# seqsense/pcgol

Hardware: AMD Instinct MI355X
Metric: Mpoints/sec ICP iter (corr+reduce) + kNN queries/sec, 1M-pt cloud (higher is better)
Workload: dtype f32

## Files before the change

pcgol_amd/csrc/icp.hip:

```cpp
#include <string.h>

#include <algorithm>
#include <array>
#include <chrono>
#include <condition_variable>
#include <mutex>
#include <string>
#include <thread>

#include <vector>

#include "knn_grid.h"
#include "knn_xwalk.h"
#include "icp_session_plan.h"
#include "icp_step_plan.h"
#include "strict_terms.h"
#include "gicp_terms.h"

namespace pcgx {

constexpr int kIcpBlock = kKnnBlock;

__device__ __forceinline__ double wave_sum_f64(double v) {
#pragma unroll
// ... 474 lines not shown
  if (kPlane) icp_plane_update_step(state, xchg, kp);
  else icp_update_step(state, xchg, kp);
}

__global__ __launch_bounds__(256) void pack_normals_kernel(const float *__restrict__ n3, int64_t n,
                                                           float4 *__restrict__ out) {
  const int64_t i = (int64_t)blockIdx.x * 256 + threadIdx.x;
  if (i < n) out[i] = make_float4(n3[3 * i], n3[3 * i + 1], n3[3 * i + 2], 0.0f);
}

__global__ __launch_bounds__(256) void pack_base_cov_kernel(const float *__restrict__ c6, int64_t n,
                                                            float4 *__restrict__ out) {
  const int64_t i = (int64_t)blockIdx.x * 256 + threadIdx.x;
  if (i >= n) return;
  out[2 * i] = make_float4(c6[6 * i], c6[6 * i + 1], c6[6 * i + 2], c6[6 * i + 3]);
  out[2 * i + 1] = make_float4(c6[6 * i + 4], c6[6 * i + 5], 0.0f, 0.0f);
}

__global__ __launch_bounds__(256) void gather_target_cov_kernel(const float *__restrict__ c6,
                                                                const int32_t *__restrict__ perm, int64_t n,
                                                                float2 *__restrict__ out) {
  const int64_t pos = (int64_t)blockIdx.x * 256 + threadIdx.x;
  if (pos >= n) return;
  const int64_t i = perm ? (int64_t)perm[pos] : pos;
  out[3 * pos] = make_float2(c6[6 * i], c6[6 * i + 1]);
  out[3 * pos + 1] = make_float2(c6[6 * i + 2], c6[6 * i + 3]);
  out[3 * pos + 2] = make_float2(c6[6 * i + 4], c6[6 * i + 5]);
}

__global__ __launch_bounds__(kGicpBlock) void icp_gicp_sums_kernel(
    const float *__restrict__ tx, const float *__restrict__ ty, const float *__restrict__ tz, int64_t nt,
    const IcpState *__restrict__ state, const float4 *__restrict__ match, const uint32_t *__restrict__ match_id,
    const float4 *__restrict__ base_cov, const float2 *__restrict__ target_cov, double *__restrict__ block_partials,
    uint32_t *__restrict__ dropped) {
  constexpr int NS = (int)P_COUNT;
  __shared__ double s_red[kGicpBlock / 64][NS];
  __shared__ uint32_t s_drop[kGicpBlock / 64];
  if (state->done) return;
  const bool project = state->iter > 0;
  float m[16];
#pragma unroll
  for (int i = 0; i < 16; i++) m[i] = project ? state->trans[i] : (i % 5 == 0 ? 1.0f : 0.0f);
  double acc[NS];
#pragma unroll
  for (int k = 0; k < NS; k++) acc[k] = 0.0;
  uint32_t n_drop = 0;
  const int64_t per = (nt + gridDim.x - 1) / gridDim.x;
  const int64_t r_begin = (int64_t)blockIdx.x * per;
  int64_t r_end = r_begin + per;
  if (r_end > nt) r_end = nt;
  for (int64_t i = r_begin + threadIdx.x; i < r_end; i += kGicpBlock) {
    const float4 bp = match[i];
    float x0 = tx[i], y0 = ty[i], z0 = tz[i];
    const float2 t0 = target_cov[3 * i], t1 = target_cov[3 * i + 1], t2 = target_cov[3 * i + 2];
    if (bp.w >= 0.0f) {
      const uint32_t id = match_id[i];
      const float4 c0 = base_cov[2 * (int64_t)id], c1 = base_cov[2 * (int64_t)id + 1];
      if (project) {
        float px, py, pz;
        mat4_transform(m, x0, y0, z0, px, py, pz);
        x0 = px; y0 = py; z0 = pz;
      }
      const float cb[6] = {c0.x, c0.y, c0.z, c0.w, c1.x, c1.y};
      const float ct[6] = {t0.x, t0.y, t1.x, t1.y, t2.x, t2.y};
      double e, g[6], H[21];
      if (gicp_terms(x0, y0, z0, bp.x, bp.y, bp.z, cb, ct, m, e, g, H)) {
        acc[P_VALUE] += e;
#pragma unroll
        for (int a = 0; a < 6; a++) acc[P_G0 + a] += g[a];
#pragma unroll
        for (int a = 0; a < 21; a++) acc[P_H0 + a] += H[a];
        acc[P_WEIGHT] += 1.0;
        acc[P_PAIRS] += 1.0;
      } else {
        n_drop++;
      }
    }
  }
  const int lane = threadIdx.x & 63, wave = threadIdx.x >> 6;
#pragma unroll
  for (int k = 0; k < NS; k++) {
    const double v = wave_sum_f64(acc[k]);
    if (lane == 0) s_red[wave][k] = v;
  }
#pragma unroll
  for (int o = 32; o > 0; o >>= 1) n_drop += __shfl_down(n_drop, o);
  if (lane == 0) s_drop[wave] = n_drop;
  __syncthreads();
  if (threadIdx.x < NS) {
    double v = 0.0;
    for (int w = 0; w < kGicpBlock / 64; w++) v += s_red[w][threadIdx.x];
    block_partials[(int64_t)blockIdx.x * NS + threadIdx.x] = v;
  }
  if (threadIdx.x == 0) {
    uint32_t d = 0;
    for (int w = 0; w < kGicpBlock / 64; w++) d += s_drop[w];
    dropped[blockIdx.x] = d;
  }
}

__global__ __launch_bounds__(256) void invert_positions_kernel(const uint32_t *__restrict__ pos_of, int64_t n,
                                                               uint32_t *__restrict__ orig_of) {
  const int64_t i = (int64_t)blockIdx.x * 256 + threadIdx.x;
  if (i < n) orig_of[pos_of[i]] = (uint32_t)i;
}

__global__ __launch_bounds__(256) void gather_soa_kernel(const float *__restrict__ q,
                                                         const int32_t *__restrict__ perm, int64_t n,
                                                         float *__restrict__ x, float *__restrict__ y,
                                                         float *__restrict__ z, uint32_t *__restrict__ pos_of) {
  const int64_t pos = (int64_t)blockIdx.x * 256 + threadIdx.x;
  if (pos >= n) return;
  const int64_t i = perm ? (int64_t)perm[pos] : pos;
  pos_of[i] = (uint32_t)pos;
  x[pos] = q[3 * i];
  y[pos] = q[3 * i + 1];
  z[pos] = q[3 * i + 2];
}

}

using namespace pcgx;

struct pcgx_icp_session {
  const pcgx_kdtree *base = nullptr;
  OwnedBlocks owned;
  bool patched = false;
  int64_t nt = 0;
  float *d_xyz = nullptr;
  IcpState *d_state = nullptr;
  double *d_partials = nullptr;
  uint32_t *d_pos_of = nullptr;
  uint32_t *d_orig_of = nullptr;
  float4 *d_match_caller = nullptr;
  bool caller_order_fresh = false;
  int strict = 0;
  bool strict_explicit = false;
  pcgx::StrictBuffers *strict_buf = nullptr;
  float *d_terms = nullptr;
  unsigned long long *d_valid = nullptr;
  int64_t nt_pad = 0;
  float4 *d_match = nullptr;
  float *d_match_cert = nullptr;
  uint32_t *d_first_leaf = nullptr;
  uint32_t *d_walk_list = nullptr;
  uint32_t *d_walk_count = nullptr;
  double *d_sums = nullptr;
  double *d_xchg = nullptr;
  int32_t steps_sharded = 0;
  int32_t host_iter = 0;
  bool spec_walk = true;
  bool spec_pending = false;
  hipStream_t spec_stream = nullptr;
  hipStream_t used[4] = {nullptr, nullptr, nullptr, nullptr};
  int n_used = 0;
  void touch(hipStream_t st) {
    for (int k = 0; k < n_used && k < 4; k++)
      if (used[k] == st) return;
    if (n_used > 0) (void)hipStreamSynchronize(used[0]);
    if (n_used < 4) used[n_used] = st;
    n_used++;
  }
  bool shard_failed = false;
  bool ring_fit_open = false;
  bool general_ready = true;
  bool small = false;
  int32_t *d_small_perm = nullptr;
  void *d_small_sync = nullptr;
  bool plane = false;
  uint32_t *d_match_id = nullptr;
  float4 *d_normals = nullptr;
  bool gicp = false;
  float4 *d_base_cov = nullptr;
  float2 *d_target_cov = nullptr;
  uint32_t *d_dropped = nullptr;
  int gicp_grid = 1;
  int n_sums() const { return plane ? (int)P_COUNT : (int)S_COUNT; }
  int grid = 1;
  IcpKernelParams kp;
  int32_t max_iteration = 20;
};

static pcgx_status settle(pcgx_icp_session *s, hipStream_t st);
static int icp_knob(const char *name, int def, int lo, int hi);

static pcgx_status enter(pcgx_icp_session *s, void *stream, hipStream_t *st) {
  *st = pick_stream(stream);
  s->touch(*st);
  return settle(s, *st);
}

template <class T>
static hipError_t session_alloc(pcgx_icp_session *s, T **p, size_t bytes) {
  const hipError_t e = dev_cache_alloc((void **)p, bytes);
  if (e == hipSuccess) s->owned.adopt(*p, dev_cache_free);
  return e;
}

static double now_us() { return std::chrono::duration<double, std::micro>(std::chrono::steady_clock::now().time_since_epoch()).count(); }

static IcpKernelParams make_kernel_params(const pcgx_icp_params *p) {
  IcpKernelParams kp;
  memset(&kp, 0, sizeof kp);
  kp.max_dist_sq = p->max_dist * p->max_dist;
  kp.min_dist_sq = p->min_dist_sq;
  kp.min_pairs = p->min_pairs == 0 ? 6 : p->min_pairs;
  kp.upd = resolve_updater(p->weight, p->threshold, p->max_iteration);
  kp.gn = resolve_gauss_newton(p->threshold, 0.0f, p->max_iteration);
  kp.weight_fn = p->weight_fn;
  kp.weight_a = p->weight_fn_param;
  return kp;
}

static int icp_grid(int64_t nt, const TreeView &tv) {
  int64_t blocks = (nt + kIcpBlock - 1) / kIcpBlock;
  int64_t cap = (int64_t)ctx().num_cu * walk_blocks_per_cu(tv) * walk_oversubscribe();
  if (blocks > cap) blocks = cap;
  if (blocks >= 8) blocks &= ~(int64_t)7;
  if (blocks < 1) blocks = 1;
  return (int)blocks;
}

struct IcpResetZero {
  uint32_t *p[3] = {nullptr, nullptr, nullptr};
  uint32_t words[3] = {0u, 0u, 0u};
};
__global__ void icp_reset_kernel(IcpState *__restrict__ state, IcpResetZero z) {
#pragma unroll
  for (int r = 0; r < 3; r++)
    for (uint32_t i = blockIdx.x * blockDim.x + threadIdx.x; i < z.words[r]; i += gridDim.x * blockDim.x) z.p[r][i] = 0u;
  if (threadIdx.x != 0 || blockIdx.x != 0) return;
  IcpState h;
  memset(&h, 0, sizeof h);
  const Mat4 id = mat4_translate(0.0f, 0.0f, 0.0f);
  for (int i = 0; i < 16; i++) h.trans[i] = id.m[i];
  *state = h;
}

static pcgx_status general_prepare(pcgx_icp_session *s, hipStream_t st) {
  if (s->general_ready) return PCGX_OK;
  const size_t n1 = (size_t)(s->nt ? s->nt : 1);
  PCGX_HIP_TRY(hipMemsetAsync(s->d_match, 0xFF, n1 * sizeof(float4), st));
  PCGX_HIP_TRY(hipMemsetAsync(s->d_match_cert, 0, n1 * sizeof(float), st));
  PCGX_HIP_TRY(hipMemsetAsync(s->d_first_leaf, 0, n1 * sizeof(uint32_t), st));
  PCGX_HIP_TRY(hipMemsetAsync(s->d_walk_count, 0, (size_t)s->grid * sizeof(uint32_t), st));
  s->general_ready = true;
  return PCGX_OK;
}

static pcgx_status reset_state(pcgx_icp_session *s, hipStream_t st) {
  IcpResetZero z;
  size_t zero_words = 0;
  if (s->spec_pending) {
    s->spec_pending = false;
    void *ptr[2];
    size_t bytes[2];
    strict_reset_ranges(s->strict_buf, ptr, bytes);
    if (s->d_walk_count) {
      z.p[0] = s->d_walk_count;
      z.words[0] = (uint32_t)s->grid;
    }
    for (int r = 0; r < 2; r++) {
      z.p[1 + r] = (uint32_t *)ptr[r];
      z.words[1 + r] = (uint32_t)(bytes[r] / sizeof(uint32_t));
    }
    for (int r = 0; r < 3; r++) zero_words += z.words[r];
  }
  const unsigned blocks = zero_words ? (unsigned)std::min<size_t>((zero_words + 1023) / 1024, 64) : 1u;
  hipLaunchKernelGGL(icp_reset_kernel, dim3(blocks), dim3(zero_words ? 256 : 64), 0, st, s->d_state, z);
  PCGX_HIP_TRY(hipGetLastError());
  s->host_iter = 0;
  if (s->shard_failed || s->steps_sharded > 0) {
    PCGX_TRY(strict_reset(s->strict_buf, st));
    s->shard_failed = false;
    s->steps_sharded = 0;
  }
  return PCGX_OK;
}

extern "C" pcgx_status pcgx_icp_session_reset(pcgx_icp_session *s, void *stream) {
  PCGX_API_LOCK();
  if (!s) return fail(PCGX_E_INVALID, "pcgx_icp_session_reset: NULL session");
  s->touch(pick_stream(stream));
  return reset_state(s, pick_stream(stream));
}

extern "C" pcgx_status pcgx_icp_session_set_pose(pcgx_icp_session *s, const float trans16[16],
                                                 int32_t iter, void *stream) {
  PCGX_API_LOCK();
  if (!s || !trans16 || iter < 0) return fail(PCGX_E_INVALID, "pcgx_icp_session_set_pose: bad argument");
  hipStream_t st;
  PCGX_TRY(enter(s, stream, &st));
  IcpState h;
  memset(&h, 0, sizeof h);
  memcpy(h.trans, trans16, sizeof h.trans);
  h.iter = iter;
  s->host_iter = 0;
  PCGX_HIP_TRY(hipMemcpyAsync(s->d_state, &h, sizeof h, hipMemcpyHostToDevice, st));
  PCGX_HIP_TRY(hipStreamSynchronize(st));
  return PCGX_OK;
}

extern "C" pcgx_status pcgx_icp_session_read_sums(pcgx_icp_session *s, double sums10[10], void *stream) {
  PCGX_API_LOCK();
  if (!s || !sums10) return fail(PCGX_E_INVALID, "pcgx_icp_session_read_sums: bad argument");
  if (s->plane) return fail(PCGX_E_INVALID, "pcgx_icp_session_read_sums: plane session (30 sums): use pcgx_icp_session_read_sums_n");
  hipStream_t st;
  PCGX_TRY(enter(s, stream, &st));
  PCGX_HIP_TRY(hipMemcpyAsync(sums10, s->d_sums, S_COUNT * sizeof(double), hipMemcpyDeviceToHost, st));
  PCGX_HIP_TRY(hipStreamSynchronize(st));
  return PCGX_OK;
}

extern "C" pcgx_status pcgx_icp_session_set_strict(pcgx_icp_session *s, int32_t on) {
  PCGX_API_LOCK();
  if (!s) return fail(PCGX_E_INVALID, "pcgx_icp_session_set_strict: NULL session");
  if (on && s->plane) return fail(PCGX_E_INVALID, "pcgx_icp_session_set_strict: point-to-plane sessions have no reference sums to reproduce");
  if (on < 0 || on > 2) return fail(PCGX_E_INVALID, "pcgx_icp_session_set_strict: mode must be 0, 1 or 2");
  if (s->spec_pending) PCGX_TRY(settle(s, s->spec_stream));
  s->strict = on;
  s->strict_explicit = on != 0;
  return PCGX_OK;
}

extern "C" pcgx_status pcgx_icp_session_sums_count(const pcgx_icp_session *s, int32_t *count) {
  PCGX_API_LOCK();
  if (!s || !count) return fail(PCGX_E_INVALID, "pcgx_icp_session_sums_count: bad argument");
  *count = s->n_sums();
  return PCGX_OK;
}

extern "C" pcgx_status pcgx_icp_session_read_sums_n(pcgx_icp_session *s, double *sums, int32_t cap, void *stream) {
  PCGX_API_LOCK();
  if (!s || !sums || cap < s->n_sums()) return fail(PCGX_E_INVALID, "pcgx_icp_session_read_sums_n: bad argument");
  hipStream_t st;
  PCGX_TRY(enter(s, stream, &st));
  PCGX_HIP_TRY(hipMemcpyAsync(sums, s->d_sums, (size_t)s->n_sums() * sizeof(double), hipMemcpyDeviceToHost, st));
  PCGX_HIP_TRY(hipStreamSynchronize(st));
  return PCGX_OK;
}

extern "C" pcgx_status pcgx_icp_session_free(pcgx_icp_session *s) {
  PCGX_API_LOCK();
  if (!s) return PCGX_OK;
  if (s->base) const_cast<pcgx_kdtree *>(s->base)->sessions.fetch_sub(1);
  if (s->n_used > 4) (void)hipDeviceSynchronize();
  else
    for (int k = 0; k < s->n_used; k++) (void)hipStreamSynchronize(s->used[k]);
  s->owned.release_all();
  delete s;
  return PCGX_OK;
}

static pcgx_status device_input(const float *src, size_t count, bool on_device, hipStream_t st, const float **d_out,
                                double *t_space = nullptr) {
  *d_out = src;
  if (on_device) return PCGX_OK;
  float *stage = nullptr;
  PCGX_TRY(ctx().arena.alloc_n(count, &stage));
  if (t_space) *t_space = now_us();
  PCGX_TRY(staged_upload(stage, src, count * sizeof(float), st));
  *d_out = stage;
  return PCGX_OK;
}

static pcgx_status setup_failed(hipError_t e) { return fail(PCGX_E_HIP, "icp session setup failed: %s", hipGetErrorString(e)); }

static pcgx_status session_allocate(pcgx_icp_session *s, const SessionPlan &p, double *d_sums) {
  void **const slot[kSessionBuffers] = {
      (void **)&s->d_xyz,        (void **)&s->d_state,      (void **)&s->d_partials,   (void **)&s->d_pos_of,
      (void **)&s->d_match,      (void **)&s->d_match_cert, (void **)&s->d_first_leaf, (void **)&s->d_walk_list,
      (void **)&s->d_walk_count, (void **)&s->d_sums,       (void **)&s->d_match_id,   (void **)&s->d_normals,
      (void **)&s->d_base_cov,   (void **)&s->d_target_cov, (void **)&s->d_dropped,    (void **)&s->d_valid,
      (void **)&s->d_small_perm};
  hipError_t e = hipSuccess;
  for (int b = 0; b < kSessionBuffers && e == hipSuccess; b++)
    if (p.bytes[b]) e = session_alloc(s, slot[b], p.bytes[b]);
  if (e == hipSuccess && p.small_buffers) e = session_alloc(s, &s->d_terms, small_fit_terms_bytes(s->nt));
  if (e == hipSuccess && p.small_buffers) e = session_alloc(s, &s->d_small_sync, small_fit_sync_bytes());
  if (e != hipSuccess) return fail(PCGX_E_OOM, "icp session allocation failed: %s", hipGetErrorString(e));
  if (d_sums) s->d_sums = d_sums;
  return PCGX_OK;
}

static pcgx_status stage_side_inputs(pcgx_icp_session *s, const float *normals, const float *base_cov6, bool on_device,
                                     hipStream_t st) {
  if (!s->plane) return PCGX_OK;
  const int64_t nb = s->base->n;
  hipError_t e;
  if (s->gicp && (e = hipMemsetAsync(s->d_dropped, 0, (size_t)s->gicp_grid * sizeof(uint32_t), st)) != hipSuccess)
    return setup_failed(e);
  PCGX_TRY(ctx().arena.begin(st));
  const float *d_in = nullptr;
  PCGX_TRY(device_input(s->gicp ? base_cov6 : normals, (size_t)nb * (s->gicp ? 6 : 3), on_device, st, &d_in));
  const dim3 blocks((unsigned)((nb + 255) / 256));
  if (s->gicp) hipLaunchKernelGGL(pack_base_cov_kernel, blocks, dim3(256), 0, st, d_in, nb, s->d_base_cov);
  else hipLaunchKernelGGL(pack_normals_kernel, blocks, dim3(256), 0, st, d_in, nb, s->d_normals);
  if ((e = hipStreamSynchronize(st)) != hipSuccess) return setup_failed(e);
  return PCGX_OK;
}

static pcgx_status order_target(pcgx_icp_session *s, const float *target, const float *target_cov6, bool on_device,
                                hipStream_t st, bool trace, double *t_phase) {
  const int64_t nt = s->nt;
  const pcgx_kdtree *base = s->base;
  Arena &ar = ctx().arena;
  PCGX_TRY(ar.begin(st));
  const float *d_q = nullptr;
  const void *up = nullptr;
  if (!on_device && s->small && (up = small_upload(target, (size_t)nt * 12)) != nullptr) {
    d_q = static_cast<const float *>(up);
    t_phase[2] = t_phase[3] = trace ? now_us() : 0.0;
  } else {
    PCGX_TRY(device_input(target, (size_t)nt * 3, on_device, st, &d_q, trace ? &t_phase[2] : nullptr));
    if (!on_device) t_phase[3] = trace ? now_us() : 0.0;
  }
  int32_t *perm = nullptr;
  if (s->small) {
    PCGX_TRY(small_fit_prepare(d_q, nt, base->bbox_lo, base->bbox_hi, s->d_small_perm, s->d_xyz, s->d_pos_of, s->d_state, s->d_terms,
                               s->d_small_sync, st));
    if (up) small_upload_read(st);
  } else {
    if (nt > 1) {
      PCGX_TRY(ar.alloc_n((size_t)nt, &perm));
      PCGX_TRY(morton_order(d_q, nt, base->bbox_lo, base->bbox_hi, perm, st));
    }
    hipLaunchKernelGGL(gather_soa_kernel, dim3((unsigned)((nt + 255) / 256)), dim3(256), 0, st, d_q, perm, nt,
                       s->d_xyz, s->d_xyz + nt, s->d_xyz + 2 * nt, s->d_pos_of);
  }
  if (s->gicp) {
    const float *d_c6 = nullptr;
    PCGX_TRY(device_input(target_cov6, (size_t)nt * 6, on_device, st, &d_c6));
    hipLaunchKernelGGL(gather_target_cov_kernel, dim3((unsigned)((nt + 255) / 256)), dim3(256), 0, st, d_c6,
                       (const int32_t *)perm, nt, s->d_target_cov);
  }
  t_phase[4] = trace ? now_us() : 0.0;
  const hipError_t e = hipGetLastError();
  return e == hipSuccess ? PCGX_OK : setup_failed(e);
}

static SessionFacts session_facts(const pcgx_kdtree *base, bool normals, bool covariances, const pcgx_icp_params *params,
                                  int64_t nt, bool caller_sums) {
  static_assert(PCGX_SUMS_REFERENCE == 0 && PCGX_SUMS_F64_TREE == 1 && S_COUNT == 10 && P_COUNT == 30,
                "SessionFacts::sums_mode, SessionPlan::n_sums");
  static const bool small_on = icp_knob("PCGX_ICP_SMALL", 1, 0, 1) != 0;
  SessionFacts f;
  f.normals = normals;
  f.covariances = covariances;
  f.sums_mode = params->sums_mode;
  if (const char *e = getenv("PCGX_ICP_STRICT")) f.strict_override = e[0] == '1' ? 1 : (e[0] == '2' ? 2 : 0);
  f.nt = nt;
  f.n_base = base->n;
  f.patched = base->n_deleted > 0;
  f.has_nan = base->has_nan;
  f.small_on = small_on;
  f.small_eligible = small_fit_eligible(base->view(), nt, base->many_ties);
  f.small_wants_order = small_fit_wants_order(nt);
  f.grid = icp_grid(nt, base->view());
  f.num_cu = ctx().num_cu;
  f.caller_sums = caller_sums;
  f.state_bytes = sizeof(IcpState);
  return f;
}

static pcgx_status session_create(const pcgx_kdtree *base, const float *normals, float damping,
                                  const float *target, int64_t nt, int32_t target_on_device,
                                  const pcgx_icp_params *params, double *d_sums,
                                  pcgx_icp_session **out, const float *base_cov6 = nullptr,
                                  const float *target_cov6 = nullptr) {
  if (!out) return fail(PCGX_E_INVALID, "pcgx_icp_session_create: out is NULL");
  *out = nullptr;
  if (!base || !params || nt < 0 || (nt > 0 && !target))
    return fail(PCGX_E_INVALID, "pcgx_icp_session_create: bad argument");
  if (params->weight_fn < 0 || params->weight_fn >= PCGX_WEIGHT_KINDS)
    return fail(PCGX_E_INVALID, "pcgx_icp_session_create: weight_fn %d is none of the built-in forms (a custom Go closure "
                                "cannot run on the device)", params->weight_fn);
  if (normals && params->weight_fn != PCGX_WEIGHT_ONE)
    return fail(PCGX_E_INVALID, "the point-to-plane extension takes the default weight only");
  if (base_cov6 && params->weight_fn != PCGX_WEIGHT_ONE)
    return fail(PCGX_E_INVALID, "the GICP extension takes the default weight only");
  if (params->sums_mode < 0 || params->sums_mode >= PCGX_SUMS_KINDS)
    return fail(PCGX_E_INVALID, "pcgx_icp_session_create: sums_mode %d is none of PCGX_SUMS_*", params->sums_mode);
  PCGX_TRY(ensure_init());
  hipStream_t st = ctx().stream;
  const bool patched = base->n_deleted > 0;
  if (patched && base->n_deleted >= base->n)
    return fail(PCGX_E_NOT_ENOUGH_PAIRS, "not enough correspondence pairs (every base point was deleted)");
  static const bool trace = getenv("PCGX_FIT_TRACE") != nullptr;
  double t_phase[6] = {0, 0, 0, 0, 0, 0};
  t_phase[0] = trace ? now_us() : 0.0;

  const SessionFacts f = session_facts(base, normals != nullptr, base_cov6 != nullptr, params, nt, d_sums != nullptr);
  const SessionPlan p = plan_session(f);

  pcgx_icp_session *s = new pcgx_icp_session();
  s->base = base;
  s->touch(st);
  s->patched = f.patched;
  const_cast<pcgx_kdtree *>(base)->sessions.fetch_add(1);
  s->nt = nt;
  s->nt_pad = p.nt_pad;
  s->gicp = p.gicp;
  s->plane = p.plane;
  s->strict = p.strict;
  s->strict_explicit = p.strict_explicit;
  s->small = p.small;
  s->grid = f.grid;
  s->gicp_grid = p.gicp_grid;
  s->kp = make_kernel_params(params);
  s->kp.gn.damping = damping;
  s->max_iteration = s->kp.upd.max_iteration;
  s->general_ready = false;

  pcgx_status rc = session_allocate(s, p, d_sums);
  if (rc == PCGX_OK) rc = stage_side_inputs(s, normals, base_cov6, target_on_device != 0, st);
  t_phase[1] = trace ? now_us() : 0.0;
  if (rc == PCGX_OK && p.start_values) rc = reset_state(s, st);
  if (rc == PCGX_OK && p.start_values) rc = general_prepare(s, st);
  if (rc == PCGX_OK && nt > 0) rc = order_target(s, target, target_cov6, target_on_device != 0, st, trace, t_phase);
  if (rc != PCGX_OK) {
    pcgx_icp_session_free(s);
    return rc;
  }
  if (trace)
    fprintf(stderr, "pcgx session trace: buffers %.0f us, memsets + arena %.0f, upload %.0f, order + gather enqueued %.0f\n",
            t_phase[1] - t_phase[0], t_phase[2] - t_phase[1], t_phase[3] - t_phase[2], t_phase[4] - t_phase[3]);
  *out = s;
  return PCGX_OK;
}

extern "C" pcgx_status pcgx_icp_session_create(const pcgx_kdtree *base, const float *target,
                                               int64_t nt, int32_t target_on_device,
                                               const pcgx_icp_params *params, double *d_sums10,
                                               pcgx_icp_session **out) {
  PCGX_API_LOCK();
  return session_create(base, nullptr, 0.0f, target, nt, target_on_device, params, d_sums10, out);
}

extern "C" pcgx_status pcgx_icp_plane_session_create(const pcgx_kdtree *base, const float *base_normals,
                                                     const float *target, int64_t nt, int32_t on_device,
                                                     const pcgx_icp_params *params, float damping,
                                                     double *d_sums30, pcgx_icp_session **out) {
  PCGX_API_LOCK();
  if (!base_normals) return fail(PCGX_E_INVALID, "pcgx_icp_plane_session_create: base_normals is NULL");
  if (params && params->min_dist_sq > 0.0f)
    return fail(PCGX_E_INVALID, "pcgx_icp_plane_session_create: MinDistSq > 0 (approximate search) is not offered here");
  if (!(damping >= 0.0f)) return fail(PCGX_E_INVALID, "pcgx_icp_plane_session_create: damping must be >= 0");
  return session_create(base, base_normals, damping, target, nt, on_device, params, d_sums30, out);
}

extern "C" pcgx_status pcgx_icp_gicp_session_create(const pcgx_kdtree *base, const float *base_cov6, const float *target,
                                                    const float *target_cov6, int64_t nt, int32_t on_device,
                                                    const pcgx_icp_params *params, float damping, double *d_sums30,
                                                    pcgx_icp_session **out) {
  PCGX_API_LOCK();
  if (!base_cov6 || (nt > 0 && !target_cov6))
    return fail(PCGX_E_INVALID, "pcgx_icp_gicp_session_create: a covariance array is NULL");
  if (params && params->min_dist_sq > 0.0f)
    return fail(PCGX_E_INVALID, "pcgx_icp_gicp_session_create: MinDistSq > 0 (approximate search) is not offered here");
  if (!(damping >= 0.0f)) return fail(PCGX_E_INVALID, "pcgx_icp_gicp_session_create: damping must be >= 0");
  return session_create(base, nullptr, damping, target, nt, on_device, params, d_sums30, out, base_cov6, target_cov6);
}

extern "C" pcgx_status pcgx_icp_gicp_session_dropped(pcgx_icp_session *s, void *stream, int64_t *n) {
  PCGX_API_LOCK();
  if (!s || !n) return fail(PCGX_E_INVALID, "pcgx_icp_gicp_session_dropped: bad argument");
  if (!s->gicp) return fail(PCGX_E_INVALID, "pcgx_icp_gicp_session_dropped: not a GICP session");
  hipStream_t st;
  PCGX_TRY(enter(s, stream, &st));
  std::vector<uint32_t> h((size_t)s->gicp_grid);
  PCGX_HIP_TRY(hipMemcpyAsync(h.data(), s->d_dropped, h.size() * sizeof(uint32_t), hipMemcpyDeviceToHost, st));
  PCGX_HIP_TRY(hipStreamSynchronize(st));
  int64_t sum = 0;
  for (uint32_t v : h) sum += (int64_t)v;
  *n = sum;
  return PCGX_OK;
}

static int icp_knob(const char *name, int def, int lo, int hi) {
  if (const char *e = getenv(name)) {
    const int v = atoi(e);
    if (v >= lo && v <= hi) return v;
  }
  return def;
}

static const StepKnobs &step_knobs() {
  static const StepKnobs knobs = [] {
    StepKnobs k;
    k.tight = icp_knob("PCGX_ICP_TIGHT", 32, 0, 32);
    k.chunks = icp_knob("PCGX_ICP_CHUNKS", 2, 1, 64);
    k.left_blocks = icp_knob("PCGX_ICP_LEFTOVER_BLOCKS", 128, 8, 4096) & ~7;
    k.cert_on = icp_knob("PCGX_ICP_CERT", 1, 0, 1) != 0;
    k.spec_on = icp_knob("PCGX_ICP_SPEC_WALK", 1, 0, 1) != 0;
    k.fused_from = icp_knob("PCGX_ICP_FUSED_FROM", 2, 0, 1 << 30);
    k.test_force_walk = icp_knob("PCGX_TEST_ICP_FORCE_WALK", 0, 0, 1 << 30);
    k.test_fused_search = icp_knob("PCGX_TEST_ICP_FUSED_SEARCH", 0, 0, 1 << 30);
    k.test_fused_grid_walk = icp_knob("PCGX_TEST_ICP_FUSED_GRID_WALK", 0, 0, 1 << 30);
    return k;
  }();
  return knobs;
}

static pcgx_status ensure_strict_buf(pcgx_icp_session *s, hipStream_t st) {
  if (s->strict_buf) return PCGX_OK;
  PCGX_TRY(strict_create(s->nt, s->d_xyz, s->d_xyz + s->nt, s->d_xyz + 2 * s->nt, (const uint32_t *)s->d_pos_of, &s->strict_buf, st));
  s->owned.adopt(s->strict_buf, [](void *p) { strict_destroy(static_cast<StrictBuffers *>(p)); });
  return PCGX_OK;
}

static pcgx_status decide_step(pcgx_icp_session *s, hipStream_t st, bool may_speculate, StepPlan *plan) {
  if (!s->patched && s->base->n_deleted > 0) s->patched = true;
  PCGX_TRY(general_prepare(s, st));
  StepFacts f;
  f.caller_had_pairs = s->caller_order_fresh;
  s->caller_order_fresh = false;
  if (!s->patched && s->strict == 1 && !s->plane && s->nt > 0) {
    if (!s->d_match_caller) {
      hipError_t e = session_alloc(s, &s->d_orig_of, (size_t)s->nt * sizeof(uint32_t));
      if (e == hipSuccess) e = session_alloc(s, &s->d_match_caller, (size_t)s->nt * sizeof(float4));
      if (e != hipSuccess) {
        (void)hipGetLastError();
        s->owned.give_up(s->d_orig_of);
        s->owned.give_up(s->d_match_caller);
        s->d_orig_of = nullptr;
        s->d_match_caller = nullptr;
      } else {
        hipLaunchKernelGGL(invert_positions_kernel, dim3((unsigned)((s->nt + 255) / 256)), dim3(256), 0, st,
                           (const uint32_t *)s->d_pos_of, s->nt, s->d_orig_of);
      }
    }
    PCGX_TRY(ensure_strict_buf(s, st));
    f.exchange = strict_work(s->strict_buf, s->kp)->exchange;
  }
  f.patched = s->patched;
  f.plane = s->plane;
  f.strict = s->strict;
  f.min_dist = s->kp.min_dist_sq > 0.0f;
  f.has_targets = s->nt > 0;
  f.grid_enabled = grid_enabled(s->base);
  f.has_cert = s->base->grid.cert != nullptr;
  f.have_match_caller = s->d_match_caller != nullptr;
  f.spec_walk = s->spec_walk;
  f.host_iter = s->host_iter;
  f.may_speculate = may_speculate;
  f.grid = s->grid;
  *plan = plan_step(f, step_knobs());
  s->caller_order_fresh = plan->next_caller_had_pairs;
  if (plan->no_walk) {
    s->spec_pending = true;
    s->spec_stream = st;
  }
  return PCGX_OK;
}

static pcgx_status enqueue_corr_patched(pcgx_icp_session *s, hipStream_t st) {
  XTreeView xv;
  PCGX_TRY(xtree_view(s->base, &xv, st));
  const size_t lds = (size_t)(xv.depth > 1 ? xv.depth : 2) * kIcpBlock * sizeof(uint32_t);
  const int64_t guard = xwalk_guard(s->base->n);
  const float *x = s->d_xyz, *y = s->d_xyz + s->nt, *z = s->d_xyz + 2 * s->nt;
  ProfScope prof(PCGX_PROF_ICP_WALK, st);
  const auto launch = [&](auto kernel) {
    hipLaunchKernelGGL(kernel, dim3(s->grid), dim3(kIcpBlock), lds, st, xv, x, y, z, s->nt, s->d_state, s->kp, s->d_match,
                       s->d_partials, s->d_match_id, (const float4 *)s->d_normals, guard);
  };
  const bool min_dist = s->kp.min_dist_sq > 0.0f;
  if (s->gicp) launch(icp_corr_xkernel<false, true, false>);
  else if (s->plane) launch(icp_corr_xkernel<false, true>);
  else if (min_dist && s->strict) launch(icp_corr_xkernel<true, false, false>);
  else if (min_dist) launch(icp_corr_xkernel<true, false>);
  else if (s->strict) launch(icp_corr_xkernel<false, false, false>);
  else launch(icp_corr_xkernel<false, false>);
  PCGX_HIP_TRY(hipGetLastError());
  return PCGX_OK;
}

static pcgx_status enqueue_corr(pcgx_icp_session *s, hipStream_t st, const StepPlan &p) {
  if (p.corr == kCorrPatched) return enqueue_corr_patched(s, st);
  if (p.corr == kCorrNone) return PCGX_OK;
  const StepKnobs &k = step_knobs();
  const float *x = s->d_xyz, *y = s->d_xyz + s->nt, *z = s->d_xyz + 2 * s->nt;
  const uint32_t *orig_of = p.write_caller ? s->d_orig_of : nullptr;
  float4 *match_caller = p.write_caller ? s->d_match_caller : nullptr;
  float *cert = p.cert ? s->d_match_cert : nullptr;
  const bool grid = p.corr != kCorrWalk;
  if (grid) {
    ProfScope prof_grid(PCGX_PROF_ICP_GRID, st);
    const bool strict_grid = s->strict && !s->plane;
    const auto launch = [&](auto kernel, int block) {
      hipLaunchKernelGGL(kernel, dim3(xcd_grid((unsigned)((s->nt + block - 1) / block))), dim3(block), 0, st, s->base->grid, x,
                         y, z, s->nt, s->d_state, s->kp, s->d_match, s->d_match_id, (const float4 *)s->d_normals,
                         s->d_first_leaf, s->d_walk_list, s->d_walk_count, (uint32_t)p.n_corr, s->d_partials,
                         (unsigned long long *)nullptr, orig_of, match_caller, cert, p.grid_has_caller_pairs ? 1 : 0,
                         p.no_walk ? 0 : 1, strict_grid ? k.test_force_walk : 0);
    };
    if (s->gicp) launch(icp_grid_kernel<true, false, false>, kIcpGridBlock);
    else if (s->plane) launch(icp_grid_kernel<true>, kIcpGridBlock);
    else if (s->strict) launch(icp_grid_kernel<false, false, false>, kIcpStrictGridBlock);
    else launch(icp_grid_kernel<false>, kIcpGridBlock);
  }
  if (p.corr == kCorrGrid) return PCGX_OK;
  ProfScope prof(grid ? PCGX_PROF_ICP_LEFTOVER : PCGX_PROF_ICP_WALK, st);
  TreeView tv = s->base->view();
  tv.tight_levels = k.tight;
  tv.chunks_per_refill = k.chunks;
  const size_t lds = walk_lds_bytes(tv, kIcpBlock);
  const StrictWork strict_w = p.tile_sums ? *strict_work(s->strict_buf, s->kp) : StrictWork();
  const auto launch = [&](auto kernel) {
    hipLaunchKernelGGL(kernel, dim3(p.n_corr), dim3(kIcpBlock), lds, st, tv, x, y, z, s->nt, s->d_state, s->kp, s->d_match,
                       s->d_first_leaf, s->d_partials, s->d_match_id, (const float4 *)s->d_normals, s->d_walk_list,
                       s->d_walk_count, (int32_t)((s->nt + kIcpGridBlock - 1) / kIcpGridBlock), orig_of, match_caller, strict_w,
                       (int32_t)(p.tile_sums ? 1 : 0), cert, s->base->grid.cert);
  };
  if (s->gicp) {
    if (grid) launch(icp_corr_kernel<false, true, true, false>);
    else launch(icp_corr_kernel<false, true, false, false>);
  } else if (s->plane) {
    if (grid) launch(icp_corr_kernel<false, true, true>);
    else launch(icp_corr_kernel<false, true, false>);
  } else if (s->kp.min_dist_sq > 0.0f) {
    if (s->strict) launch(icp_corr_kernel<true, false, false, false>);
    else launch(icp_corr_kernel<true, false, false>);
  } else if (s->strict) {
    if (grid) launch(icp_corr_kernel<false, false, true, false>);
    else launch(icp_corr_kernel<false, false, false, false>);
  } else {
    if (grid) launch(icp_corr_kernel<false, false, true>);
    else launch(icp_corr_kernel<false, false, false>);
  }
  return PCGX_OK;
}

struct StrictPairs {
  const float4 *match;
  const uint32_t *pos_of;
};
static StrictPairs strict_pairs(const pcgx_icp_session *s, bool caller_order) {
  if (caller_order) return {s->d_match_caller, nullptr};
  return {s->d_match, s->d_pos_of};
}

template <bool kFuseUpdate>
static pcgx_status enqueue_sums(pcgx_icp_session *s, hipStream_t st, const StepPlan &p) {
  if (s->strict == 1) {
    PCGX_TRY(ensure_strict_buf(s, st));
    s->host_iter++;
    CertifiedTerms C;
    if (p.certify) {
      C.grid = s->base->grid;
      C.max_dist_sq = s->kp.max_dist_sq;
      C.match_caller = s->d_match_caller;
      C.match = s->d_match;
      C.match_cert = s->d_match_cert;
      C.pos_of = s->d_pos_of;
      C.test_force_walk = step_knobs().test_fused_search;
      C.test_force_grid_walk = step_knobs().test_fused_grid_walk;
    }
    const StrictPairs pairs = strict_pairs(s, p.sums_caller);
    PCGX_TRY(strict_enqueue(s->strict_buf, pairs.match, pairs.pos_of, s->d_state, s->d_sums, s->kp, kFuseUpdate,
                            p.have_tile_sums, p.first_iter, st, p.certify ? &C : nullptr));
  } else if (s->strict) {
    if (!s->d_terms) {
      s->nt_pad = (s->nt + 63) & ~(int64_t)63;
      const size_t np = (size_t)(s->nt_pad ? s->nt_pad : 64);
      PCGX_HIP_TRY(session_alloc(s, &s->d_terms, 9 * np * sizeof(float)));
      PCGX_HIP_TRY(session_alloc(s, &s->d_valid, (np / 64) * sizeof(unsigned long long)));
    }
    PCGX_TRY(strict_check_enqueue(s->d_xyz, s->nt, s->nt_pad, (const float4 *)s->d_match, (const uint32_t *)s->d_pos_of,
                                  s->d_state, s->kp, s->d_terms, s->d_valid, s->d_sums, kFuseUpdate, st));
  } else if (s->gicp) {
    const float *x = s->d_xyz, *y = s->d_xyz + s->nt, *z = s->d_xyz + 2 * s->nt;
    hipLaunchKernelGGL(icp_gicp_sums_kernel, dim3(s->gicp_grid), dim3(kGicpBlock), 0, st, x, y, z, s->nt, s->d_state,
                       (const float4 *)s->d_match, (const uint32_t *)s->d_match_id, (const float4 *)s->d_base_cov,
                       (const float2 *)s->d_target_cov, s->d_partials, s->d_dropped);
    hipLaunchKernelGGL((icp_final_reduce_kernel<kFuseUpdate, true>), dim3(1), dim3(1024), 0, st, s->d_partials,
                       s->gicp_grid, s->d_state, s->d_sums, s->kp);
  } else if (s->plane)
    hipLaunchKernelGGL((icp_final_reduce_kernel<kFuseUpdate, true>), dim3(1), dim3(1024), 0, st, s->d_partials, s->grid,
                       s->d_state, s->d_sums, s->kp);
  else
    hipLaunchKernelGGL((icp_final_reduce_kernel<kFuseUpdate, false>), dim3(1), dim3(64 * S_COUNT), 0, st, s->d_partials,
                       s->grid, s->d_state, s->d_sums, s->kp);
  PCGX_HIP_TRY(hipGetLastError());
  return PCGX_OK;
}

template <bool kFuseUpdate>
static pcgx_status enqueue_step(pcgx_icp_session *s, hipStream_t st, bool may_speculate) {
  StepPlan plan;
  PCGX_TRY(decide_step(s, st, may_speculate, &plan));
  PCGX_TRY(enqueue_corr(s, st, plan));
  return enqueue_sums<kFuseUpdate>(s, st, plan);
}

static pcgx_status settle(pcgx_icp_session *s, hipStream_t st) {
  if (!s->spec_pending) return PCGX_OK;
  s->spec_pending = false;
  IcpState h;
  PCGX_HIP_TRY(hipMemcpyAsync(&h, s->d_state, sizeof h, hipMemcpyDeviceToHost, st));
  PCGX_HIP_TRY(hipStreamSynchronize(st));
  if (h.done != 2) return PCGX_OK;
  s->spec_walk = false;
  const int32_t missing = s->host_iter - h.num_iteration;
  if (getenv("PCGX_ICP_SPEC_TRACE"))
    fprintf(stderr, "pcgx icp: a step without the leftover walk met a target the grid could not answer: %d of %d Evaluates enqueued again, with the walk\n",
            (int)missing, (int)s->host_iter);
  const int32_t zero = 0;
  PCGX_HIP_TRY(hipMemcpyAsync(&s->d_state->done, &zero, sizeof zero, hipMemcpyHostToDevice, st));
  PCGX_HIP_TRY(hipMemsetAsync(s->d_walk_count, 0, (size_t)s->grid * sizeof(uint32_t), st));
  PCGX_TRY(strict_reset(s->strict_buf, st));
  s->host_iter = h.num_iteration;
  for (int32_t k = 0; k < missing; k++) PCGX_TRY(enqueue_step<true>(s, st, false));
  PCGX_HIP_TRY(hipGetLastError());
  return PCGX_OK;
}

extern "C" pcgx_status pcgx_debug_icp_strict_stats(pcgx_icp_session *s, void *stream, int64_t out[64]) {
  PCGX_API_LOCK();
  if (!s || !out) return fail(PCGX_E_INVALID, "pcgx_debug_icp_strict_stats: NULL argument");
  for (int k = 0; k < 64; k++) out[k] = 0;
  if (!s->strict_buf) return PCGX_OK;
  PCGX_TRY(settle(s, pick_stream(stream)));
  unsigned long long h[64];
  PCGX_TRY(strict_read_debug(s->strict_buf, h, pick_stream(stream)));
  for (int k = 0; k < 64; k++) out[k] = (int64_t)h[k];
  return PCGX_OK;
}

extern "C" pcgx_status pcgx_icp_session_partials(pcgx_icp_session *s, void *stream) {
  PCGX_API_LOCK();
  if (!s) return fail(PCGX_E_INVALID, "pcgx_icp_session_partials: NULL session");
  hipStream_t st;
  PCGX_TRY(enter(s, stream, &st));
  return enqueue_step<false>(s, st, false);
}

extern "C" pcgx_status pcgx_icp_session_update(pcgx_icp_session *s, void *stream) {
  PCGX_API_LOCK();
  if (!s) return fail(PCGX_E_INVALID, "pcgx_icp_session_update: NULL session");
  hipStream_t st;
  PCGX_TRY(enter(s, stream, &st));
  if (s->plane)
    hipLaunchKernelGGL(icp_update_kernel<true>, dim3(1), dim3(64), 0, st, s->d_state, s->d_sums, s->kp);
  else
    hipLaunchKernelGGL(icp_update_kernel<false>, dim3(1), dim3(64), 0, st, s->d_state, s->d_sums, s->kp);
  PCGX_HIP_TRY(hipGetLastError());
  return PCGX_OK;
}

static bool small_now(const pcgx_icp_session *s) {
  return s->small && s->strict == 1 && !s->plane && !s->patched && s->base->n_deleted == 0 && !s->spec_pending &&
         !(s->kp.max_dist_sq < s->kp.min_dist_sq);
}
static pcgx_status small_steps(pcgx_icp_session *s, hipStream_t st, int iters, uint32_t *mail_seq = nullptr) {
  s->caller_order_fresh = false;
  s->host_iter += iters;
  static std::atomic<uint32_t> launches{0};
  static std::mutex one_at_a_time;
  static hipEvent_t last_done[16] = {};
  std::lock_guard<std::mutex> lk(one_at_a_time);
  const int slot = current_slot() & 15;
  if (!last_done[slot]) PCGX_HIP_TRY(hipEventCreateWithFlags(&last_done[slot], hipEventDisableTiming));
  else PCGX_HIP_TRY(hipStreamWaitEvent(st, last_done[slot], 0));
  struct Record {
    hipEvent_t ev;
    hipStream_t st;
    ~Record() { (void)hipEventRecord(ev, st); }
  } record{last_done[slot], st};
  while (iters > 0) {
    const int now = iters < small_fit_max_iters() ? iters : small_fit_max_iters();
    const bool mail = mail_seq != nullptr && iters == now && ctx().mailbox != nullptr;
    if (mail) *mail_seq = mailbox_next_seq();
    PCGX_TRY(small_fit_enqueue(s->base->view(), s->d_xyz, s->d_xyz + s->nt, s->d_xyz + 2 * s->nt, s->nt, s->d_state, s->kp, s->d_terms,
                               s->d_valid, s->d_sums, s->d_small_sync, ++launches, now, s->d_small_perm, st, mail ? ctx().mailbox : nullptr,
                               mail ? *mail_seq : 0u));
    iters -= now;
  }
  return PCGX_OK;
}

extern "C" pcgx_status pcgx_icp_session_step(pcgx_icp_session *s, void *stream) {
  PCGX_API_LOCK();
  if (!s) return fail(PCGX_E_INVALID, "pcgx_icp_session_step: NULL session");
  hipStream_t st = pick_stream(stream);
  s->touch(st);
  if (small_now(s)) return small_steps(s, st, 1);
  return enqueue_step<true>(s, st, true);
}

static pcgx_status step_sharded_impl(pcgx_icp_session *s, pcgx_comm *c, void *stream, pcgx_status *local_rc) {
  int32_t rank = 0, world = 1;
  PCGX_TRY(pcgx_comm_rank(c, &rank, &world));
  hipStream_t st;
  PCGX_TRY(enter(s, stream, &st));
  const int step = s->steps_sharded++;
  if (step == 0 && world > 1 && s->strict == 1 && !s->plane && !s->ring_fit_open) comm_ring_new_fit(c);
  s->ring_fit_open = false;
  if (const char *e = getenv("PCGX_TEST_FAIL_RANK")) {
    const char *it = getenv("PCGX_TEST_FAIL_ITER");
    if (atoi(e) == rank && it && atoi(it) == step && !s->shard_failed) {
      *local_rc = fail(PCGX_E_HIP, "injected failure of rank %d in iteration %d (PCGX_TEST_FAIL_RANK)", rank, step);
      s->shard_failed = true;
    }
  }
  const bool reference = s->strict == 1 && !s->plane;
  if (reference) {
    RingView ring;
    const bool have_ring = comm_ring_step(c, step, &ring);
    if (!s->shard_failed) {
      StepPlan plan;
      pcgx_status rc = decide_step(s, st, false, &plan);
      if (rc == PCGX_OK) rc = enqueue_corr(s, st, plan);
      if (rc != PCGX_OK) {
        *local_rc = rc;
        s->shard_failed = true;
      }
    }
    PCGX_TRY(ensure_strict_buf(s, st));
    const StrictPairs pairs = strict_pairs(s, s->caller_order_fresh);
    if (have_ring) {
      const bool first_iter = s->host_iter++ == 0;
      return strict_enqueue_ring(s->strict_buf, pairs.match, pairs.pos_of, s->d_state, s->d_sums, s->kp, ring, s->shard_failed,
                                 first_iter, st);
    }
    return strict_enqueue_sharded(s->strict_buf, pairs.match, pairs.pos_of, s->d_state, s->d_sums, s->kp, c, rank, world,
                                  s->shard_failed, st);
  }
  const int n = s->n_sums();
  if (!s->d_xchg) {
    if (session_alloc(s, &s->d_xchg, (size_t)(n + 2) * sizeof(double)) != hipSuccess)
      return fail(PCGX_E_OOM, "pcgx_icp_session_step_sharded: no memory for the exchange");
  }
  PCGX_HIP_TRY(hipMemsetAsync(s->d_xchg, 0, (size_t)(n + 2) * sizeof(double), st));
  if (!s->shard_failed) {
    double *keep = s->d_sums;
    s->d_sums = s->d_xchg;
    const pcgx_status rc = pcgx_icp_session_partials(s, stream);
    s->d_sums = keep;
    if (rc != PCGX_OK) {
      *local_rc = rc;
      s->shard_failed = true;
    }
  }
  if (s->shard_failed) {
    static const double one = 1.0;
    PCGX_HIP_TRY(hipMemcpyAsync(s->d_xchg + n, &one, sizeof one, hipMemcpyHostToDevice, st));
  }
  PCGX_TRY(pcgx_comm_allreduce_f64(c, s->d_xchg, n + 1, stream));
// ... 444 lines not shown
```

pcgol_amd/csrc/icp_step_plan.h:

```cpp
#pragma once
#include <cstdint>

namespace pcgx {

struct StepFacts {
  bool patched = false;
  bool plane = false;
  int32_t strict = 0;
  bool min_dist = false;
  bool has_targets = false;
  bool grid_enabled = false;
  bool has_cert = false;
  bool have_match_caller = false;
  bool caller_had_pairs = false;
  bool exchange = false;
  bool spec_walk = true;
  int32_t host_iter = 0;
  bool may_speculate = false;
  int32_t grid = 1;
};

struct StepKnobs {
  int32_t tight = 32;
  int32_t chunks = 2;
  int32_t left_blocks = 128;
  bool cert_on = true;
  bool spec_on = true;
  int32_t fused_from = 2;
  int32_t test_force_walk = 0;
  int32_t test_fused_search = 0;
  int32_t test_fused_grid_walk = 0;
};

enum CorrForm : int32_t {
  kCorrPatched = 0,
  kCorrWalk = 1,
  kCorrGridWalk = 2,
  kCorrGrid = 3,
  kCorrNone = 4,
};

struct StepPlan {
  CorrForm corr = kCorrWalk;
  int32_t n_corr = 1;
  bool write_caller = false;
  bool tile_sums = false;
  bool grid_has_caller_pairs = false;
  bool cert = false;
  bool no_walk = false;
  bool certify = false;
  bool sums_caller = false;
  bool have_tile_sums = false;
  bool first_iter = false;
  bool next_caller_had_pairs = false;
};

inline StepPlan plan_step(const StepFacts &f, const StepKnobs &k) {
  StepPlan p;
  p.n_corr = f.grid;
  p.first_iter = f.host_iter == 0;
  if (f.patched) {
    p.corr = kCorrPatched;
    return p;
  }
  const bool caller = f.strict == 1 && !f.plane && f.has_targets && f.have_match_caller;
  p.write_caller = p.sums_caller = p.next_caller_had_pairs = caller;
  const bool grid = f.grid_enabled && !f.min_dist && f.has_targets;
  p.tile_sums = p.have_tile_sums = grid && caller && !f.exchange;
  if (grid && f.strict && !f.plane && f.grid > k.left_blocks) p.n_corr = k.left_blocks;
  p.cert = grid && k.cert_on && f.has_cert;
  p.grid_has_caller_pairs = grid && f.strict && !f.plane && f.caller_had_pairs;
  p.no_walk = f.may_speculate && k.spec_on && f.spec_walk && grid && f.strict == 1 && !f.plane && f.host_iter >= 1 &&
              !p.tile_sums;
  p.certify = p.no_walk && k.fused_from > 0 && f.host_iter >= k.fused_from && p.cert && f.caller_had_pairs && caller &&
              f.exchange;
  p.corr = p.certify ? kCorrNone : p.no_walk ? kCorrGrid : grid ? kCorrGridWalk : kCorrWalk;
  return p;
}

}
```

pcgol_amd/csrc/pcgx_internal.h:

```cpp
#pragma once
#include <hip/hip_runtime.h>
#include <stdint.h>
#include <stdio.h>
#include <stdlib.h>

#include <atomic>
#include <memory>
#include <mutex>
#include <string>
#include <utility>
#include <vector>

#include "../../include/pcgx.h"
#include "pcgx_math.h"

namespace pcgx {

template <class T>
struct DefaultInitAlloc : std::allocator<T> {
  template <class U>
  struct rebind {
    using other = DefaultInitAlloc<U>;
  };
  template <class U>
// ... 133 lines not shown
  int32_t d = 0;
  while (n > 0) { d++; n >>= 1; }
  return d;
}

pcgx_status build_tree_device(const float *d_xyz, int64_t n, int32_t depth, uint32_t *d_order, float4 *d_nodes,
                              const int32_t *d_labels, hipStream_t st);

}
pcgx_status resolve_tree(const pcgx_kdtree *t, const pcgx_kdtree **active, bool *empty);
void xtree_delete(pcgx_kdtree *t, int64_t pid);
void xtree_delete_batch(pcgx_kdtree *t, const int64_t *ids, int64_t m);
void xtree_free(pcgx_kdtree *t);
int xtree_max_depth(const pcgx_kdtree *t);
int64_t xtree_host_walk_max();
long long xtree_host_walks(bool reset);
void xtree_host_nearest(const pcgx_kdtree *t, const float *q, int64_t nq, float max_range, float min_dist_sq, int64_t *ids,
                        float *dist_sq);
bool xtree_host_range(const pcgx_kdtree *t, const float *q, int64_t nq, float max_range, int64_t *counts, const int64_t *offsets,
                      int64_t *ids, float *dist_sq);
pcgx_status xtree_launch_nearest(const pcgx_kdtree *t, const float *d_q, const int32_t *d_perm, int64_t nq,
                                 float max_range_sq, float min_dist_sq, int32_t *d_ids, float *d_dsq, hipStream_t st);
namespace pcgx {

constexpr int kKnnBlock = 512;
constexpr int kWalkQueueBytesPerWave = 7 * 128 * 4;
inline size_t walk_stack_bytes(const TreeView &tv, int block) {
  int levels = tv.depth > 1 ? tv.depth - 1 : 1;
  return (size_t)levels * block * sizeof(uint32_t);
}
#ifndef PCGX_WALK_TOP_LEVELS
#define PCGX_WALK_TOP_LEVELS 6
#endif
constexpr int kWalkTopLevels = PCGX_WALK_TOP_LEVELS;
constexpr int kWalkTopBytes = (1 << kWalkTopLevels) * 4;
inline size_t walk_lds_bytes(const TreeView &tv, int block) {
  return walk_stack_bytes(tv, block) + (size_t)(block / 64) * kWalkQueueBytesPerWave + kWalkTopBytes;
}
int walk_blocks_per_cu(const TreeView &tv);
int walk_refill_threshold();
int walk_tight_levels();
int walk_chunks_per_refill();
int walk_oversubscribe();
pcgx_status launch_nearest(const TreeView &tv, const float *d_q, const int32_t *d_perm, int64_t nq,
                           float max_range_sq, float min_dist_sq, int32_t *d_ids, float *d_dsq,
                           hipStream_t st);
pcgx_status launch_nearest_listed(const TreeView &tv, const float *d_q, const int32_t *d_list,
                                  const uint32_t *d_count, int64_t nq_max, float max_range_sq, int32_t *d_ids,
                                  float *d_dsq, hipStream_t st);

size_t radix_sort_workspace_bytes(int64_t n);
pcgx_status radix_sort_pairs(uint32_t *keys[2], uint32_t *vals[2], int64_t n, int key_bits,
                             void *workspace, int *result, hipStream_t st, bool iota_vals = false,
                             bool first_hist_done = false);
struct RadixFirstHist {
  uint32_t *hist;
  int nblocks, items;
};
RadixFirstHist radix_first_hist(int64_t n, void *workspace);
pcgx_status launch_minmax(const void *d_data, int64_t n, int32_t stride, int32_t off, float *d_out6,
                          hipStream_t st, bool sticky_first = true);
constexpr size_t kTicketBytes = 8192;
constexpr size_t kMailboxBytes = 2048;
pcgx_status read_back_small(const void *d_src, size_t bytes, void *host_dst, hipStream_t st);
uint32_t mailbox_next_seq();
pcgx_status mailbox_wait(uint32_t seq, size_t bytes, void *host_dst, hipStream_t st);
pcgx_status mailbox_wait_tagged(uint32_t seq, int words, uint32_t *host_dst, hipStream_t st);
pcgx_status minmax_to_host(const void *d_data, int64_t n, int32_t stride, int32_t off, float *d_out6, float out6[6],
                           hipStream_t st, bool sticky_first = true);
pcgx_status morton_order(const float *d_q, int64_t n, const float lo[3], const float hi[3], int32_t *d_perm,
                         hipStream_t st);

struct IcpState {
  float trans[16];
  int32_t iter;
  int32_t num_iteration;
  int32_t done;
  int32_t status;
  Evaluated ev;
  float hessian[36];
};


struct IcpKernelParams {
  float max_dist_sq;
  float min_dist_sq;
  int32_t min_pairs;
  UpdaterParams upd;
  GaussNewtonParams gn;
  int32_t weight_fn;
  float weight_a;
};


#if defined(__HIPCC__)
constexpr unsigned int kTicketGroups = 32u, kTicketStride = 32u;
static_assert((1u + kTicketGroups) * kTicketStride * 4u <= kTicketBytes, "the context's ticket words");
__device__ __forceinline__ bool last_workgroup_ticket(unsigned int *tickets) {
  const unsigned int g = blockIdx.x & (kTicketGroups - 1u), groups = min(gridDim.x, kTicketGroups);
  const unsigned int members = (gridDim.x - g + kTicketGroups - 1u) / kTicketGroups;
  unsigned int *mine = tickets + kTicketStride * (1u + g);
  if (atomicAdd(mine, 1u) != members - 1u) return false;
  __hip_atomic_store(mine, 0u, __ATOMIC_RELAXED, __HIP_MEMORY_SCOPE_AGENT);
  if (atomicAdd(tickets, 1u) != groups - 1u) return false;
  __hip_atomic_store(tickets, 0u, __ATOMIC_RELAXED, __HIP_MEMORY_SCOPE_AGENT);
  return true;
}

__device__ __forceinline__ uint32_t wave_incl_scan_u32(uint32_t v) {
#define PCGX_DPP_ADD(CTRL, MASK) v += (uint32_t)__builtin_amdgcn_update_dpp(0, (int)v, CTRL, MASK, 0xf, (MASK) == 0xf)
  PCGX_DPP_ADD(0x111, 0xf);
  PCGX_DPP_ADD(0x112, 0xf);
  PCGX_DPP_ADD(0x114, 0xf);
  PCGX_DPP_ADD(0x118, 0xf);
  PCGX_DPP_ADD(0x142, 0xa);
  PCGX_DPP_ADD(0x143, 0xc);
#undef PCGX_DPP_ADD
  return v;
}
__device__ __forceinline__ void icp_update_step(IcpState *__restrict__ state, const double *__restrict__ sums10,
                                                const IcpKernelParams &kp, const float *pose_in = nullptr,
                                                const int32_t *count_in = nullptr) {
  state->num_iteration = (count_in ? count_in[1] : state->num_iteration) + 1;
  const int64_t npairs = (int64_t)sums10[S_PAIRS];
  if (npairs < (int64_t)kp.min_pairs) {
    state->ev.num_pairs = npairs;
    state->status = PCGX_E_NOT_ENOUGH_PAIRS;
    state->done = 1;
    return;
  }
  Evaluated ev;
  finish_evaluate(sums10, ev);
  state->ev = ev;
  Mat4 t;
  for (int i = 0; i < 16; i++) t.m[i] = pose_in ? pose_in[i] : state->trans[i];
  int32_t it = count_in ? count_in[0] : state->iter;
  const bool converged = gradient_descent_update(kp.upd, it, ev.gradient, t);
  for (int i = 0; i < 16; i++) state->trans[i] = t.m[i];
  state->iter = it;
  if (converged) state->done = 1;
}

#endif

struct StrictBuffers;
struct StrictWork;
struct CertifiedTerms;
pcgx_status strict_create(int64_t nt, const float *tx, const float *ty, const float *tz, const uint32_t *pos_of,
                          StrictBuffers **out, hipStream_t st);
void strict_destroy(StrictBuffers *b);
const StrictWork *strict_work(StrictBuffers *b, const IcpKernelParams &kp);
pcgx_status strict_enqueue(StrictBuffers *b, const float4 *match, const uint32_t *pos_of, IcpState *state,
                           double *sums10, const IcpKernelParams &kp, bool fuse_update, bool have_tile_sums, bool first_iter,
                           hipStream_t st, const struct CertifiedTerms *certify = nullptr);
pcgx_status strict_read_debug(StrictBuffers *b, unsigned long long out[64], hipStream_t st);
pcgx_status strict_check_enqueue(const float *d_xyz, int64_t nt, int64_t nt_pad, const float4 *match, const uint32_t *pos_of,
                                 IcpState *state, const IcpKernelParams &kp, float *d_terms, unsigned long long *d_valid,
                                 double *d_sums, bool fuse_update, hipStream_t st);
pcgx_status strict_enqueue_sharded(StrictBuffers *b, const float4 *match, const uint32_t *pos_of, IcpState *state,
                                   double *sums10, const IcpKernelParams &kp, pcgx_comm *c, int rank, int world,
                                   bool local_failed, hipStream_t st);
struct RingView {
  unsigned long long *words = nullptr;
  unsigned long long *host = nullptr;
  unsigned long long *const *tab = nullptr;
  unsigned long long *mine = nullptr;
  int32_t words_per_rank = 0, rank = 0, world = 1;
  uint32_t epoch = 0;
  int32_t kind = 0;
  long long guess_ticks = 0;
};
pcgx_status strict_enqueue_ring(StrictBuffers *b, const float4 *match, const uint32_t *pos_of, IcpState *state, double *sums10,
                                const IcpKernelParams &kp, const RingView &ring, bool local_failed, bool first_iter, hipStream_t st);
void ring_abort_from_host(const RingView &ring, uint32_t reason);
pcgx_status strict_reset(StrictBuffers *b, hipStream_t st);
void strict_reset_ranges(StrictBuffers *b, void *ptr[2], size_t bytes[2]);
bool small_fit_eligible(const TreeView &tv, int64_t nt, bool many_ties);
size_t small_fit_sync_bytes();
size_t small_fit_terms_bytes(int64_t nt);
int small_fit_max_iters();
bool small_fit_wants_order(int64_t nt);
pcgx_status small_fit_prepare(const float *d_target_aos, int64_t nt, const float box_lo[3], const float box_hi[3], int32_t *d_perm, float *d_xyz,
                               uint32_t *d_pos_of, IcpState *state, void *terms, void *sync, hipStream_t st);
pcgx_status small_fit_enqueue(const TreeView &tv, const float *tx, const float *ty, const float *tz, int64_t nt, IcpState *state,
                              const IcpKernelParams &kp, void *terms, unsigned long long *valid, double *sums10, void *sync,
                              uint32_t launch_no, int iters, const int32_t *perm, hipStream_t st, volatile uint32_t *mailbox = nullptr,
                              uint32_t mailbox_seq = 0u);
bool comm_ring_step(pcgx_comm *c, int32_t step, RingView *out);
void comm_ring_new_fit(pcgx_comm *c);
int comm_ring_kind(pcgx_comm *c);
void comm_attach_local_ring(pcgx_comm *c, unsigned long long *block, int32_t words_per_rank);
}

struct pcgx_kdtree {
  int64_t n = 0;
  int32_t depth = 0;
  float4 *d_nodes = nullptr;
  uint32_t *d_dir = nullptr;
  uint32_t *d_inv = nullptr;
  int32_t dir_bits = 0;
  float dir_lo[3] = {0, 0, 0}, dir_scale[3] = {0, 0, 0};
  float bbox_lo[3] = {0, 0, 0}, bbox_hi[3] = {0, 0, 0};
  bool has_nan = false;
  bool many_ties = false;
  pcgx::RawVector<int32_t> inorder;
  pcgx::RawVector<float> points;
  struct XNode {
    int32_t id, c0, c1, dim;
  };
  pcgx::RawVector<XNode> xnodes;
  int32_t xroot = -1;
  bool x_init = false, x_dirty = false;
  float4 *d_xpts = nullptr;
  void *d_xlinks = nullptr;
  float *d_xsrc = nullptr;
  std::vector<uint8_t> xsub;
  float4 *d_gpts = nullptr;
  uint32_t *d_gstart = nullptr;
  float *d_gcert = nullptr;
  pcgx::GridView grid;
  bool grid_ok = false;
  double grid_crowding = 0.0;
  std::vector<uint8_t> deleted;
  int64_t n_deleted = 0;
  bool dirty = false;
  pcgx_kdtree *live = nullptr;
  std::vector<pcgx_kdtree *> retired;
  std::atomic<int> sessions{0};
  std::mutex mu;
  pcgx::TreeView view() const {
    pcgx::TreeView v;
    v.nodes = d_nodes;
    v.n = (int32_t)n;
    v.depth = depth;
    v.dir = d_dir;
    v.dir_bits = dir_bits;
    for (int k = 0; k < 3; k++) { v.dir_lo[k] = dir_lo[k]; v.dir_scale[k] = dir_scale[k]; }
    v.refill_threshold = pcgx::walk_refill_threshold();
    v.tight_levels = pcgx::walk_tight_levels();
    v.chunks_per_refill = pcgx::walk_chunks_per_refill();
    return v;
  }
};
```

pcgol_amd/csrc/strict.hip:

```cpp
#include <stddef.h>

#include "knn_grid.h"
#include "strict_plan.h"
#include "strict_terms.h"

namespace pcgx {

__device__ __forceinline__ int lane_next(int v, int edge) { return __builtin_amdgcn_update_dpp(edge, v, 0x130, 0xf, 0xf, false); }
__device__ __forceinline__ int lane_prev(int v, int edge) { return __builtin_amdgcn_update_dpp(edge, v, 0x138, 0xf, 0xf, false); }
__device__ __forceinline__ double wave_excl_scan_f64(double v, int lane) {
  double inc = v;
  inc += dpp_f64<0x111, 0xf>(0.0, inc);
  inc += dpp_f64<0x112, 0xf>(0.0, inc);
  inc += dpp_f64<0x114, 0xf>(0.0, inc);
  inc += dpp_f64<0x118, 0xf>(0.0, inc);
  inc += dpp_f64<0x142, 0xa>(0.0, inc);
  inc += dpp_f64<0x143, 0xc>(0.0, inc);
  (void)lane;
  return dpp_f64<0x138, 0xf>(0.0, inc);
}
__device__ __forceinline__ uint32_t wave_all_umin(uint32_t v) {
#define PCGX_DPP_U32(CTRL, MASK) (uint32_t) __builtin_amdgcn_update_dpp(-1, (int)v, CTRL, MASK, 0xf, false)
  v = umin(v, PCGX_DPP_U32(0x111, 0xf));
  v = umin(v, PCGX_DPP_U32(0x112, 0xf));
// ... 250 lines not shown
  out[3 * i + 2] = tz[pos];
}

__device__ __forceinline__ uint32_t serial_leaf_regs(uint32_t s, const float *t, int l) {
  float x = u2f(s);
#pragma unroll
  for (int j = 0; j < kLeaf; j++) x = x + u2f((uint32_t)__builtin_amdgcn_readlane((int)f2u(t[j]), l));
  return f2u(x);
}

__device__ __forceinline__ void tile_guesses(const LdsQuads &q, double base, double lsum, double pre, int lane, uint32_t &g,
                                             ChainRange &cr, double &tile_err) {
  g = f2u((float)(base + pre));
  const float e = u2f(plain_chain_q(q, g));
  const double err = ((double)e - (double)u2f(g)) - lsum;
  const double epre = wave_excl_scan_f64(err, lane);
  tile_err = lane_f64(epre, 63) + lane_f64(err, 63);
  const uint32_t g2 = f2u((float)(base + pre + epre));
  const int32_t moved = (int32_t)g2 - (int32_t)g;
  if (__ballot(moved > 2 || moved < -2) != 0ull) g = g2;
  cr = guess_chain_q(q, g);
}
__device__ __forceinline__ void tile_guesses_pair(const LdsQuads &q, double base, double lsum, double pre, int lane, uint32_t &g,
                                                  ChainRange &cr, ChainRange &crb, double &tile_err) {
  g = f2u((float)(base + pre));
  const float e = u2f(plain_chain_q(q, g));
  const double err = ((double)e - (double)u2f(g)) - lsum;
  const double epre = wave_excl_scan_f64(err, lane);
  tile_err = lane_f64(epre, 63) + lane_f64(err, 63);
  const uint32_t g2 = f2u((float)(base + pre + epre));
  const int32_t moved = (int32_t)g2 - (int32_t)g;
  if (__ballot(moved > 2 || moved < -2) != 0ull) g = g2;
  guess_chain_pair_q(q, g, cr, crb);
}

constexpr int kExactTiles = 1;
constexpr uint32_t kPlainMargin = 512u;
constexpr uint32_t kMaybeMargin = 1u << 17;

constexpr int kSumBlock = 512;
constexpr int kSumWaves = kSumBlock / 64;
enum { JOB_CROSSING = 1, JOB_NOWINDOW = 2 };

constexpr long long kExchangeTicks = 200000;
__device__ __forceinline__ int nth_set_bit(unsigned long long m, int n) {
  int pos = 0;
#pragma unroll
  for (int w = 32; w > 0; w >>= 1) {
    const int cnt = __popcll(m & (((1ull << w) - 1ull) << pos));
    const bool up = n >= cnt;
    n -= up ? cnt : 0;
    pos += up ? w : 0;
  }
  return pos;
}

struct CertifiedStore {
  float4 best;
  float best_d;
  uint32_t pos;
  int32_t q;
};
__device__ __forceinline__ void certified_store_flush(const CertifiedTerms &C, int64_t tile, CertifiedStore &D) {
  if (D.q < 0) return;
  const bool found = __float_as_int(D.best.w) >= 0;
  const float cert = (D.q & 0x10000) ? C.grid.cert[__float_as_uint(D.best.w)] : 0.0f;
  const int64_t c = tile * kTile + (D.q & 0xffff);
  C.match[D.pos] = make_float4(D.best.x, D.best.y, D.best.z, found ? D.best_d : -1.0f);
  C.match_cert[D.pos] = cert;
  C.match_caller[c] = make_float4(D.best.x, D.best.y, D.best.z, found ? cert : -1.0f);
  D.q = -1;
}

__device__ __forceinline__ int certified_wave_search(const CertifiedTerms &C, const IcpState *state, const StrictWork &W, int64_t tile,
                                                      int lane, int wave, const bool (&fail)[4], float (&mx)[4], float (&my)[4],
                                                      float (&mz)[4], const float (&ub)[4], float4 (&bp)[4], float4 *park,
                                                      CertifiedStore &D) {
  constexpr int kStride = kTile / 4;
  unsigned long long m[4];
  int base[5];
  base[0] = 0;
#pragma unroll
  for (int c = 0; c < 4; c++) {
    m[c] = __ballot(fail[c]);
    base[c + 1] = base[c] + __popcll(m[c]);
  }
  const int n = base[4];
  if (n == 0) return 0;
#pragma unroll 1
  for (int r0 = 0; r0 < n; r0 += kLanes) {
    certified_store_flush(C, tile, D);
    const bool on = r0 + lane < n;
    const int k = on ? r0 + lane : r0;
    const int c = (k >= base[1] ? 1 : 0) + (k >= base[2] ? 1 : 0) + (k >= base[3] ? 1 : 0);
    const unsigned long long mc = c == 0 ? m[0] : (c == 1 ? m[1] : (c == 2 ? m[2] : m[3]));
    const int bc = c == 0 ? base[0] : (c == 1 ? base[1] : (c == 2 ? base[2] : base[3]));
    const int owner = nth_set_bit(mc, k - bc);
    float x = 0.0f, y = 0.0f, z = 0.0f, u = 0.0f;
#pragma unroll
    for (int cc = 0; cc < 4; cc++) {
      const float gx = __shfl(mx[cc], owner), gy = __shfl(my[cc], owner), gz = __shfl(mz[cc], owner), gu = __shfl(ub[cc], owner);
      x = c == cc ? gx : x;
      y = c == cc ? gy : y;
      z = c == cc ? gz : z;
      u = c == cc ? gu : u;
    }
#pragma unroll
    for (int cc = 0; cc < 4; cc++) park[cc * kStride] = bp[cc];
    park[4 * kStride] = make_float4(mx[0], mx[1], mx[2], mx[3]);
    park[5 * kStride] = make_float4(my[0], my[1], my[2], my[3]);
    park[6 * kStride] = make_float4(mz[0], mz[1], mz[2], mz[3]);
    float4 best = make_float4(0.0f, 0.0f, 0.0f, __int_as_float(-1));
    float best_d = C.max_dist_sq;
    float w_new = -1.0f;
    __builtin_amdgcn_s_setprio(3);
    if (on) {
      const int q = 4 * (wave * kLanes + owner) + c;
      const int64_t cg = tile * kTile + q;
      const uint32_t pos = C.pos_of[cg];
      GridVerdict v = grid_nearest(C.grid, x, y, z, C.max_dist_sq, u, best, best_d);
      if (C.test_force_grid_walk && cg % C.test_force_grid_walk == 0) v = GRID_WALK;
      if (v == GRID_WALK) {
        if (atomicCAS(&const_cast<IcpState *>(state)->done, 0, 2) == 0) atomicAdd(&W.dbg[47], 1ull << 32);
      } else {
        const bool found = __float_as_int(best.w) >= 0;
        w_new = found ? best_d : -1.0f;
        D.best = best;
        D.best_d = best_d;
        D.pos = pos;
        D.q = q | ((v == GRID_FOUND && found) ? 0x10000 : 0);
      }
    }
    __builtin_amdgcn_s_setprio(0);
    float4 *back = park;
    asm volatile("" : "+v"(back));
#pragma unroll
    for (int cc = 0; cc < 4; cc++) bp[cc] = back[cc * kStride];
    const float4 px = back[4 * kStride], py = back[5 * kStride], pz = back[6 * kStride];
    mx[0] = px.x; mx[1] = px.y; mx[2] = px.z; mx[3] = px.w;
    my[0] = py.x; my[1] = py.y; my[2] = py.z; my[3] = py.w;
    mz[0] = pz.x; mz[1] = pz.y; mz[2] = pz.z; mz[3] = pz.w;
#pragma unroll
    for (int cc = 0; cc < 4; cc++) {
      const int src = base[cc] + __popcll(m[cc] & ((1ull << lane) - 1ull)) - r0;
      const bool got = ((m[cc] >> lane) & 1ull) && src >= 0 && src < kLanes;
      const int sl = got ? src : lane;
      const float rx = __shfl(best.x, sl), ry = __shfl(best.y, sl), rz = __shfl(best.z, sl), rw = __shfl(w_new, sl);
      if (got) bp[cc] = make_float4(rx, ry, rz, rw);
    }
  }
  return n;
}

template <bool kExchange, bool kSharded = false, bool kCertify = false>
__global__ __launch_bounds__(kSumBlock) __attribute__((amdgpu_waves_per_eu(4, 4))) void strict_sum_kernel(
    const float4 *__restrict__ match, const uint32_t *__restrict__ pos_of, const IcpState *__restrict__ state, StrictWork W,
    CertifiedTerms C = CertifiedTerms()) {
  __shared__ float4 s_terms[kStrictRows][kTile / 4];
  __shared__ int s_np[kSumWaves];
  __shared__ int s_ns[kCertify ? kSumWaves : 1];
  __shared__ double s_tot[16];
  static_assert(!kSharded || kExchange, "the ring form rides on the exchange");
  static_assert(!kCertify || (kExchange && !kSharded), "the certified terms: one GPU, with the exchange");
  const int done = state->done;
  const int lane = threadIdx.x & 63, wave = threadIdx.x >> 6;
  const int64_t tile = blockIdx.x;
  const int NR = W.nrows;
  const long long t_0 = trace_clock(W);
  long long t_x0 = 0;
  CertifiedStore held;
  held.q = -1;
  double P0 = (!kExchange && wave < NR) ? tile_prefix(W.tile_sum, W.ntiles, wave, tile, lane) : 0.0;
  {
    const TermSrc S = make_term_src(match, pos_of, state, W);
    const int l = threadIdx.x >> 3, v = threadIdx.x & 7;
    float4 bp[4];
    float tx[4], ty[4], tz[4];
    const int64_t i0 = tile * kTile + (int64_t)l * kLeaf + 4 * v;
    load_quad(S, i0, bp, tx, ty, tz);
    float t[4][kStrictRows];
    int np = 0;
    if (kCertify) {
      bool fail[4];
      float ub[4];
#pragma unroll
      for (int c = 0; c < 4; c++) {
        float x = tx[c], y = ty[c], z = tz[c];
        if (S.project) mat4_transform(S.m, tx[c], ty[c], tz[c], x, y, z);
        const float dx = bp[c].x - x, dy = bp[c].y - y, dz = bp[c].z - z;
        const float dm = (dx * dx + dy * dy) + dz * dz;
        bool kept = S.project && bp[c].w >= 0.0f && dm < bp[c].w && dm < C.max_dist_sq;
        if ((C.test_force_walk && (i0 + c) % C.test_force_walk == 0) || (C.test_force_grid_walk && (i0 + c) % C.test_force_grid_walk == 0))
          kept = false;
        fail[c] = !kept && i0 + c < W.nt;
        ub[c] = (S.project && bp[c].w >= 0.0f && dm == dm) ? dm : __builtin_inff();
        if (fail[c]) bp[c].w = -1.0f;
        tx[c] = x; ty[c] = y; tz[c] = z;
      }
      int ns = 0;
      if (!done) ns = certified_wave_search(C, state, W, tile, lane, wave, fail, tx, ty, tz, ub, bp, &s_terms[0][tile_quad(l, v)], held);
      if (lane == 0) s_ns[wave] = ns;
      TermSrc S0 = S;
      S0.project = false;
#pragma unroll
      for (int c = 0; c < 4; c++) np += pair_terms(S0, tx[c], ty[c], tz[c], bp[c], t[c]) ? 1 : 0;
    } else {
#pragma unroll
      for (int c = 0; c < 4; c++) np += pair_terms(S, tx[c], ty[c], tz[c], bp[c], t[c]) ? 1 : 0;
    }
#pragma unroll
    for (int k = 0; k < kStrictRows; k++) s_terms[k][tile_quad(l, v)] = make_float4(t[0][k], t[1][k], t[2][k], t[3][k]);
#pragma unroll
    for (int o = 32; o > 0; o >>= 1) np += __shfl_xor(np, o);
    if (lane == 0) s_np[wave] = np;
  }
  __syncthreads();
  const long long t_p1 = trace_clock(W);
  if (done) return;
  if (threadIdx.x == 0) {
    int np = 0;
    for (int w = 0; w < kSumWaves; w++) np += s_np[w];
    W.tile_pairs[tile] = (uint32_t)np;
  }
  static_assert(kStrictRows <= 2 * kSumWaves, "a wave has at most two rows");
  double lsum_kept[2] = {0.0, 0.0}, pre_kept[2] = {0.0, 0.0};
  if (kExchange) {
#pragma unroll
    for (int pass = 0; pass < 2; pass++) {
      const int row = wave + pass * kSumWaves;
      if (row >= NR) break;
      const LdsQuads q{s_terms[row], lane};
      double lsum = 0.0;
#pragma unroll
      for (int v = 0; v < kLeaf / 4; v++) {
        const float4 a = q(v);
        lsum += (double)a.x; lsum += (double)a.y; lsum += (double)a.z; lsum += (double)a.w;
      }
      const double pre = wave_excl_scan_f64(lsum, lane);
      lsum_kept[pass] = lsum;
      pre_kept[pass] = pre;
      if (lane == 63) s_tot[row] = pre + lsum;
    }
    __syncthreads();
    t_x0 = trace_clock(W);
    if (wave == 0) {
      if (lane < NR) {
        const double v = s_tot[lane];
        __hip_atomic_store(&W.tile_pub[(int64_t)lane * W.ntiles_pad + tile], v, __ATOMIC_RELAXED, __HIP_MEMORY_SCOPE_AGENT);
        W.tile_sum[(int64_t)lane * W.ntiles + tile] = v;
      }
      asm volatile("s_waitcnt vmcnt(0)" ::: "memory");
      const int64_t g_mine = tile >> 5, n_groups = (W.ntiles + 31) >> 5;
      if (lane == 0) {
        const uint32_t bit = 1u << (tile & 31);
        const uint32_t full = (g_mine == n_groups - 1 && (W.ntiles & 31)) ? (1u << (W.ntiles & 31)) - 1u : 0xffffffffu;
        const uint32_t old = __hip_atomic_fetch_or(&W.tile_arrived[32 * g_mine], bit, __ATOMIC_RELAXED, __HIP_MEMORY_SCOPE_AGENT);
        if ((old | bit) == full)
          __hip_atomic_fetch_or(&W.tile_arrived[32 * (n_groups + (g_mine >> 5))], 1u << (g_mine & 31), __ATOMIC_RELAXED,
                                __HIP_MEMORY_SCOPE_AGENT);
      }
      bool gave_up = false;
      const int64_t G_mine = g_mine >> 5;
      long long t_first = 0;
      for (int64_t G0 = 0; G0 <= G_mine && !gave_up; G0 += kLanes - 1) {
        const int64_t G = G0 + lane - 1;
        uint32_t want = 0u;
        const unsigned int *word = W.tile_arrived;
        if (lane == 0) {
          want = G0 == 0 ? (1u << (tile & 31)) - 1u : 0u;
          word = W.tile_arrived + 32 * g_mine;
        } else if (G <= G_mine) {
          want = G < G_mine ? 0xffffffffu : (1u << (g_mine & 31)) - 1u;
          word = W.tile_arrived + 32 * (n_groups + G);
        }
        for (int spins = 0;; spins++) {
          uint32_t have = 0u;
          if (want) have = __hip_atomic_load(word, __ATOMIC_RELAXED, __HIP_MEMORY_SCOPE_AGENT);
          if (__ballot((have & want) != want) == 0ull) break;
          if ((spins & 63) == 63) {
            const long long now = (long long)wall_clock64();
            if (t_first == 0) t_first = now;
            if (now - t_first > kExchangeTicks) {
              gave_up = true;
              break;
            }
          }
          __builtin_amdgcn_s_sleep(4);
        }
      }
      if (gave_up && lane == 0) atomicAdd(&W.dbg[63], 1ull);
      if (kSharded && W.rank > 0) {
        if (tile == 0) {
          const RingLayout RL{W.world};
          double acc = 0.0;
          for (int k0 = 0; k0 < W.rank; k0 += 7) {
            const int k = k0 + lane / kStrictRows, row = lane % kStrictRows;
            double v = 0.0;
            if (lane < 7 * kStrictRows && k < W.rank && row < NR) (void)ring_wait_f64(W, RL.row_tot(k, row), v, W.ring_guess_ticks);
#pragma unroll
            for (int j = 0; j < 7; j++) {
              const double vj = __shfl(v, j * kStrictRows + (lane < kStrictRows ? lane : 0));
              acc += vj;
            }
          }
          if (lane < NR) __hip_atomic_store(&W.ring_base[lane], acc, __ATOMIC_RELAXED, __HIP_MEMORY_SCOPE_AGENT);
          asm volatile("s_waitcnt vmcnt(0)" ::: "memory");
          if (lane == 0) __hip_atomic_store(W.ring_flag, W.ring_epoch, __ATOMIC_RELAXED, __HIP_MEMORY_SCOPE_AGENT);
        } else {
          long long t_first = 0;
          for (int spins = 0;; spins++) {
            if (__hip_atomic_load(W.ring_flag, __ATOMIC_RELAXED, __HIP_MEMORY_SCOPE_AGENT) == W.ring_epoch) break;
            if ((spins & 63) == 63) {
              const long long now = (long long)wall_clock64();
              if (t_first == 0) t_first = now;
              if (now - t_first > 2 * W.ring_guess_ticks) break;
            }
            __builtin_amdgcn_s_sleep(4);
          }
        }
      }
    }
    __syncthreads();
  }
  const long long t_1 = trace_clock(W);
  for (int row = wave; row < NR; row += kSumWaves) {
    if (kExchange) P0 = tile_prefix_pub(W.tile_pub, W.ntiles_pad, row, tile, lane);
    else if (row >= kSumWaves) P0 = tile_prefix(W.tile_sum, W.ntiles, row, tile, lane);
    double P0r = P0 + ((!kSharded && W.row_base) ? W.row_base[row] : 0.0);
    if (kSharded) {
      if (W.rank > 0) P0r = P0 + __hip_atomic_load(&W.ring_base[row], __ATOMIC_RELAXED, __HIP_MEMORY_SCOPE_AGENT);
      if (tile == W.ntiles - 1 && lane < W.world - 1 - W.rank) {
        const RingLayout RL{W.world};
        ring_put_f64(ring_inbox(W, W.rank + 1 + lane) + RL.row_tot(W.rank, row), P0 + s_tot[row], W.ring_epoch);
      }
    }
    const LdsQuads q{s_terms[row], lane};
    TileRec T;
    T.s = summary_identity();
    T.key = -1;
    T.in = T.out = 0u;
    T.cons = 0;
    const bool first = tile < kExactTiles && W.first_exact;
    double lsum = 0.0, pre;
    if (kExchange) {
      lsum = row < kSumWaves ? lsum_kept[0] : lsum_kept[1];
      pre = row < kSumWaves ? pre_kept[0] : pre_kept[1];
    } else {
#pragma unroll
      for (int v = 0; v < kLeaf / 4; v++) {
        const float4 a = q(v);
        lsum += (double)a.x; lsum += (double)a.y; lsum += (double)a.z; lsum += (double)a.w;
      }
      pre = wave_excl_scan_f64(lsum, lane);
    }
    uint32_t g;
    ChainRange cr, crb;
    double terr;
    tile_guesses_pair(q, P0r, lsum, pre, lane, g, cr, crb, terr);
    const double tile_total = lane_f64(pre, 63) + lane_f64(lsum, 63);
    if (lane == 0)
      W.tile_err[(int64_t)row * W.ntiles + tile] = terr + (tile_total - (kExchange ? s_tot[row] : W.tile_sum[(int64_t)row * W.ntiles + tile]));
    const uint32_t mn = wave_all_umin(cr.mn), mx = wave_all_umax(cr.mx);
    const bool one_sign = __ballot(cr.sg_or != cr.sg_and) == 0ull &&
                          (__ballot(cr.sg_or != 0u) == 0ull || __ballot(cr.sg_or == 0u) == 0ull);
    const uint32_t g_first = (uint32_t)rfl((int)g);
    const int32_t key = one_sign ? choose_window(mn, mx, g_first >> 31, g_first & 0x7fffffffu) : -1;
    const uint32_t g_next = (uint32_t)lane_next((int)g, (int)g);
    const bool cons = __ballot(lane < 63 && g_next != cr.end) == 0ull;
    T.key = key;
    T.in = g_first;
    T.out = (uint32_t)__builtin_amdgcn_readlane((int)cr.end, 63);
    T.cons = cons ? 1 : 0;
    const uint32_t m_lo = mn & 0x7fffffu, m_hi = mx & 0x7fffffu;
    int32_t maybe_E = -1;
    if (!first && key >= 0 && (mn >> 23) == (mx >> 23) && m_lo >= kPlainMargin && m_hi <= 0x7fffffu - kPlainMargin) {
      const uint32_t E = mn >> 23;
      Par S = leaf_parity_summary_pair(g, cr, crb, E, g_first >> 31);
      auto fold = [&](const Par &Y, int o) {
        if ((lane & (2 * o - 1)) == 0) S = par_compose(S, Y);
      };
#define PCGX_PAR_DPP(CTRL, O)                                                                         \
  do {                                                                                                \
    Par Y;                                                                                            \
    _Pragma("unroll") for (int p = 0; p < 2; p++) {                                                   \
      Y.c[p] = dpp_partner<CTRL, 0xf>(S.c[p]);                    \
      Y.lo[p] = dpp_partner<CTRL, 0xf>(S.lo[p]);                 \
      Y.hi[p] = dpp_partner<CTRL, 0xf>(S.hi[p]);                 \
    }                                                                                                 \
    fold(Y, O);                                                                                       \
  } while (0)
      PCGX_PAR_DPP(0x101, 1);
      PCGX_PAR_DPP(0x102, 2);
      PCGX_PAR_DPP(0x104, 4);
      PCGX_PAR_DPP(0x108, 8);
#undef PCGX_PAR_DPP
#pragma unroll
      for (int o = 16; o < 64; o <<= 1) {
        Par Y;
#pragma unroll
        for (int p = 0; p < 2; p++) {
          Y.c[p] = __shfl(S.c[p], lane + o);
          Y.lo[p] = __shfl(S.lo[p], lane + o);
          Y.hi[p] = __shfl(S.hi[p], lane + o);
        }
        fold(Y, o);
      }
      T.s = par_expand(S, E, key);
      if (lane == 0) W.recs[row * W.ntiles + tile] = T;
      maybe_E = (m_lo < kMaybeMargin || m_hi > 0x7fffffu - kMaybeMargin) ? (int32_t)E : -1;
      if (maybe_E < 0) continue;
    }
    unsigned slot = 0xffffffffu;
    const unsigned shard = (unsigned)((tile + 7 * row) % kAuxShards), per_shard = (unsigned)W.naux / kAuxShards;
    if (lane == 0) {
      const unsigned k = atomicAdd(&W.aux_count[shard * 32], 1u);
      slot = k < per_shard ? shard * per_shard + k : 0xffffffffu;
    }
    slot = (unsigned)rfl((int)slot);
    if (slot == 0xffffffffu) {
      if (maybe_E < 0) {
        T.key = -1;
        T.cons = 0;
        if (lane == 0) W.recs[row * W.ntiles + tile] = T;
      }
      continue;
    }
    if (lane == 0) {
      JobDesc *J = W.jobs + slot;
      J->row = row;
      J->tile = tile;
      J->pad = maybe_E >= 0 ? (1 | (maybe_E << 8)) : 0;
    }
    float4 *dst = W.aux_terms + (size_t)slot * (kTile / 4);
    int lane_here = lane;
    asm volatile("" : "+v"(lane_here));
#pragma unroll
    for (int v = 0; v < kLeaf / 4; v++) dst[v * kLanes + lane_here] = s_terms[row][v * kLanes + lane_here];
  }
  if (kCertify) {
    certified_store_flush(C, tile, held);
    if (threadIdx.x == 0) {
      if (tile == 0) atomicAdd(&W.dbg[47], 1ull);
      int ns = 0;
      for (int w = 0; w < kSumWaves; w++) ns += s_ns[w];
      if (ns > 0) atomicAdd(&W.dbg[59], (unsigned long long)ns);
    }
  }
  if (threadIdx.x == 0 && (W.selfcheck & 2)) {
    W.stamps[tile * 16 + 0] = (unsigned long long)t_0;
    W.stamps[tile * 16 + 1] = (unsigned long long)t_1;
    W.stamps[tile * 16 + 2] = (unsigned long long)t_x0;
    W.stamps[tile * 16 + 3] = (unsigned long long)t_p1;
    W.stamps[tile * 16 + 5] = (unsigned long long)trace_clock(W);
  }
}

constexpr int kJobBlock = 256;
constexpr int kJobRoles = 3;
template <bool kRegs>
__device__ __forceinline__ uint32_t resolve_staged(uint32_t s, int kind, int32_t key, const LeafAux &A, int lane,
                                               const float4 *lds, const float *t, int &serial_out, int &tried_out,
                                               int &applied_out);
__global__ __launch_bounds__(kJobBlock) void strict_job_kernel(const IcpState *__restrict__ state, StrictWork W) {
  __shared__ float4 s_t[kTile / 4];
  __shared__ float4 s_lin[kTile / 4];
  __shared__ int32_t s_S[12][kLanes];
  __shared__ uint32_t s_g[kLanes];
  __shared__ int32_t s_lk[kLanes];
  __shared__ int32_t s_hdr[5];
  __shared__ uint32_t s_ctab[4][kCandInner];
  __shared__ int s_cdone, s_pieces;
  const unsigned per_shard = (unsigned)W.naux / kAuxShards;
  const int lane = threadIdx.x & 63, part = threadIdx.x >> 6;
  const int role = (int)(blockIdx.x % kJobRoles);
  const unsigned jb = blockIdx.x / kJobRoles;
  const unsigned shard = jb % kAuxShards, slot = shard * per_shard + jb / kAuxShards;
  const JobDesc *J = W.jobs + slot;
  const float4 *src4 = W.aux_terms + (size_t)slot * (kTile / 4);
  static_assert(kTile / 4 == 2 * kJobBlock, "two quads of the tile per thread");
  const bool early = jb / kAuxShards < 6;
  float4 q0 = make_float4(0.0f, 0.0f, 0.0f, 0.0f), q1 = q0;
  int row = 0, pad = 0;
  int64_t tile = 0;
  if (early) {
    q0 = src4[threadIdx.x];
    q1 = src4[threadIdx.x + kJobBlock];
    row = J->row;
    tile = J->tile;
    pad = J->pad;
  }
  const int done = state->done;
  const unsigned handed_out = W.aux_count[shard * 32];
  if (done || slot % per_shard >= min(handed_out, per_shard)) return;
  if (threadIdx.x == 0) s_cdone = s_pieces = 0;
  if (!early) {
    q0 = src4[threadIdx.x];
    q1 = src4[threadIdx.x + kJobBlock];
    row = J->row;
    tile = J->tile;
    pad = J->pad;
  }
  {
    int i = threadIdx.x;
    s_t[i] = q0;
    s_lin[8 * ((i & 63) ^ (i >> 6)) + (i >> 6)] = q0;
    i += kJobBlock;
    s_t[i] = q1;
    s_lin[8 * ((i & 63) ^ (i >> 6)) + (i >> 6)] = q1;
  }
  const long long tj_0 = trace_clock(W);
  __syncthreads();
  const long long tj_1 = trace_clock(W);
  auto stamp_end = [&](int what) {
    if ((W.selfcheck & 2) && lane == 0) {
      W.stamps[tile * 16 + 6] = (unsigned long long)tj_0;
      W.stamps[tile * 16 + 7] = (unsigned long long)tj_1;
      atomicMax(&W.stamps[tile * 16 + 8 + (part >= 4 ? 1 : 0)], (unsigned long long)trace_clock(W));
      W.stamps[tile * 16 + 10] = (unsigned long long)(what | (row << 8));
    }
  };
  const bool first = tile < kExactTiles && W.first_exact;
  if (first && role != 0) return;
  const bool traced = (W.selfcheck & 2) && part == 0 && !first && tile > kStrictRows;
  auto stage = [&](int word, uint32_t dep) {
    if (traced) {
      const unsigned long long tt = clock_after(dep);
      if (lane == 0) W.stamps[tile * 16 + word] = tt;
    }
  };
  if (part == 0) {
    const LdsQuads q{s_t, lane};
    double lsum = 0.0;
#pragma unroll
    for (int v = 0; v < kLeaf / 4; v++) {
      const float4 a = q(v);
      lsum += (double)a.x; lsum += (double)a.y; lsum += (double)a.z; lsum += (double)a.w;
    }
    const double pre = wave_excl_scan_f64(lsum, lane);
    const double base = tile_prefix2(W.tile_sum, W.tile_err, W.ntiles, row, tile, lane) +
                        (W.row_base ? W.row_base[row] + W.err_base[row] : 0.0);
    uint32_t g;
    ChainRange cr;
    double terr;
    tile_guesses(q, base, lsum, pre, lane, g, cr, terr);
    const uint32_t mn = wave_all_umin(cr.mn), mx = wave_all_umax(cr.mx);
    const bool one_sign = __ballot(cr.sg_or != cr.sg_and) == 0ull &&
                          (__ballot(cr.sg_or != 0u) == 0ull || __ballot(cr.sg_or == 0u) == 0ull);
    const uint32_t g_first = (uint32_t)rfl((int)g);
    const int32_t key = (one_sign && !first) ? choose_window(mn, mx, g_first >> 31, g_first & 0x7fffffffu) : -1;
    const uint32_t g_next = (uint32_t)lane_next((int)g, (int)g);
    const bool cons = __ballot(lane < 63 && g_next != cr.end) == 0ull;
    s_g[lane] = g;
    s_lk[lane] = key >= 0 ? key : leaf_key(cr, g);
    const uint32_t out_last = (uint32_t)__builtin_amdgcn_readlane((int)cr.end, 63);
    const uint32_t m_lo = mn & 0x7fffffu, m_hi = mx & 0x7fffffu;
    const bool stands = (pad & 1) && key >= 0 && (mn >> 23) == (mx >> 23) && (int32_t)(mn >> 23) == (pad >> 8) &&
                        m_lo >= kPlainMargin && m_hi <= 0x7fffffu - kPlainMargin;
    stage(11, g ^ (uint32_t)key);
    if (lane == 0) {
      s_hdr[0] = key;
      s_hdr[1] = (int32_t)g_first;
      s_hdr[2] = (int32_t)out_last;
      s_hdr[3] = cons ? 1 : 0;
      s_hdr[4] = stands ? 1 : 0;
    }
  }
  __syncthreads();
  if (s_hdr[4]) { if (part == 0 && role == 0) stamp_end(4); return; }
  const uint32_t g = s_g[lane];
  const int32_t lk = s_lk[lane];
  const int32_t tkey = s_hdr[0];
  const int kind = tkey >= 0 ? JOB_CROSSING : JOB_NOWINDOW;
  if (part < 4 && role == 0) {
    int32_t c, lo, hi;
    leaf_class_piece_q(LdsQuads{s_t, lane}, g, lk, part, c, lo, hi);
    s_S[part][lane] = c;
    s_S[4 + part][lane] = lo;
    s_S[8 + part][lane] = hi;
    stage(12, (uint32_t)(c ^ lo ^ hi));
    lds_fence_wave();
    if (lane == 0) __hip_atomic_fetch_add(&s_pieces, 1, __ATOMIC_RELEASE, __HIP_MEMORY_SCOPE_WORKGROUP);
  }
  const bool scans = role == 0 && (part == 0 || (part == 1 && kind == JOB_CROSSING));
  if (scans)
    while (__hip_atomic_load(&s_pieces, __ATOMIC_ACQUIRE, __HIP_MEMORY_SCOPE_WORKGROUP) < 4) __builtin_amdgcn_s_sleep(1);
  if (first && part >= 1) return;
  if (kind == JOB_NOWINDOW && (role != 0 || part >= 1)) {
    if (role == 0) return;
    constexpr int kPer = 2, kWavesNw = kCand / (kPer * kLanes);
    static_assert(kWavesNw * kPer * kLanes == kCand && kWavesNw <= (kJobRoles - 1) * (kJobBlock / 64), "roles 1, 2 carry the table");
    const int wave_nw = (role - 1) * (kJobBlock / 64) + part;
    if (wave_nw >= kWavesNw) return;
    const uint32_t g0 = (uint32_t)s_hdr[1];
    const uint32_t mag = g0 & 0x7fffffffu;
    uint32_t out[kPer];
// ... 354 lines not shown
__device__ __forceinline__ TileRec rec_get(const RecArray &a, int i) {
  TileRec R;
  R.key = a[0][i]; R.in = (uint32_t)a[1][i]; R.out = (uint32_t)a[2][i]; R.cons = a[3][i];
#pragma unroll
  for (int q = 0; q < 4; q++) {
    R.s.c[q] = a[4 + q][i];
    R.s.lo[q] = a[8 + q][i];
    R.s.hi[q] = a[12 + q][i];
  }
  return R;
}
__device__ __forceinline__ TileRec load_rec_uniform(const RecArray &a, int i) {
  const TileRec V = rec_get(a, i);
  TileRec R;
  R.key = rfl(V.key); R.in = (uint32_t)rfl((int)V.in); R.out = (uint32_t)rfl((int)V.out); R.cons = rfl(V.cons);
#pragma unroll
  for (int q = 0; q < 4; q++) {
    R.s.c[q] = rfl(V.s.c[q]);
    R.s.lo[q] = rfl(V.s.lo[q]);
    R.s.hi[q] = rfl(V.s.hi[q]);
  }
  return R;
}

__device__ __forceinline__ TileRec shfl_rec(const TileRec &R, int src) {
  TileRec X;
  X.key = __shfl(R.key, src);
  X.in = (uint32_t)__shfl((int)R.in, src);
  X.out = (uint32_t)__shfl((int)R.out, src);
  X.cons = __shfl(R.cons, src);
  X.s = shfl_summary(R.s, src);
  return X;
}
template <int kCtrl, int kRowMask>
__device__ __forceinline__ int dpp_int(int v) {
  return dpp_partner<kCtrl, kRowMask>(v);
}
template <int kCtrl, int kRowMask>
__device__ __forceinline__ TileRec dpp_rec(const TileRec &R) {
  TileRec X;
  X.key = dpp_int<kCtrl, kRowMask>(R.key);
  X.in = (uint32_t)dpp_int<kCtrl, kRowMask>((int)R.in);
  X.out = (uint32_t)dpp_int<kCtrl, kRowMask>((int)R.out);
  X.cons = dpp_int<kCtrl, kRowMask>(R.cons);
#pragma unroll
  for (int q = 0; q < 4; q++) {
    X.s.c[q] = dpp_int<kCtrl, kRowMask>(R.s.c[q]);
    X.s.lo[q] = dpp_int<kCtrl, kRowMask>(R.s.lo[q]);
    X.s.hi[q] = dpp_int<kCtrl, kRowMask>(R.s.hi[q]);
  }
  return X;
}
__device__ __forceinline__ TileRec compose_rec(const TileRec &X, const TileRec &Y) {
  TileRec Z;
  Z.key = Y.key;
  Z.s = compose(X.s, Y.s);
  Z.cons = ((X.cons & 1) && (Y.cons & 1) && X.out == Y.in) ? 1 : 0;
  Z.in = X.in;
  Z.out = Y.out;
  return Z;
}

#ifndef PCGX_NARROW_RECORD
#define PCGX_NARROW_RECORD 64
#endif
constexpr int32_t kNarrowRecord = PCGX_NARROW_RECORD;
__device__ __forceinline__ bool stands_alone(const TileRec &R) {
  if (kNarrowRecord <= 0 || R.key < 0 || (R.cons >> 8) == 0) return false;
  int32_t w = kBig;
#pragma unroll
  for (int r = 0; r < 4; r++) {
    const int32_t d = R.s.hi[r] - R.s.lo[r];
    w = d >= 0 ? imin(w, d) : w;
  }
  return w < kNarrowRecord || w == kBig;
}

__device__ __forceinline__ int lds_get(const int *p) { return __hip_atomic_load(p, __ATOMIC_ACQUIRE, __HIP_MEMORY_SCOPE_WORKGROUP); }
__device__ __forceinline__ void lds_put(int *p, int v) { __hip_atomic_store(p, v, __ATOMIC_RELEASE, __HIP_MEMORY_SCOPE_WORKGROUP); }

struct ChainMail {
  int req;
  int ack;
  uint32_t s_in, s_out;
};

template <bool kCheck, bool kSpec = false>
__global__ __launch_bounds__(kChainBlock) void strict_chain_kernel(const float4 *__restrict__ match,
                                                                  const uint32_t *__restrict__ pos_of,
                                                                  IcpState *__restrict__ state, StrictWork W,
                                                                  double *__restrict__ sums10, IcpKernelParams kp,
                                                                  int fuse_update) {
  __shared__ RecArray s_rec;
  __shared__ RecArray s_pre;
  __shared__ RecArray s_suf;
  __shared__ int16_t s_tail[kChainTiles];
  __shared__ int16_t s_head[kChainTiles];
  __shared__ int16_t s_auxlist[kChainTiles];
  __shared__ int16_t s_auxord[kChainTiles];
  __shared__ int32_t s_count[kChainSegs], s_auxcnt[kChainSegs];
  __shared__ uint32_t s_auxmask[kChainSegs][2];
  __shared__ int s_sufok[kChainSegs];
  __shared__ int s_pre_cnt[2];
  __shared__ int s_progress;
  __shared__ ChainMail s_mail[kChainSegs];
  __shared__ uint32_t s_tab[kTabSlots][kCand];
  __shared__ int s_tab_ord[kTabSlots];
  __shared__ float4 s_tile[kTile / 4];
  __shared__ unsigned long long s_np;
  __shared__ int s_np_ok;
  __shared__ uint32_t s_stat[8];
  __shared__ unsigned long long s_wk[8];
  __shared__ unsigned long long s_stat_ticks[2];
  __shared__ float s_pose[16];
  __shared__ int32_t s_pose_n[2];
  const int done = state->done;
  const int row = (int)(blockIdx.x % (unsigned)W.nrows), my_chunk = (int)(blockIdx.x / (unsigned)W.nrows);
  const int lane = threadIdx.x & 63, wave = rfl((int)(threadIdx.x >> 6));
  const bool walker = wave == kWalker;
  const bool last_chunk = my_chunk == W.nchunks - 1;
  auto term_src = [&]() { return make_term_src(match, pos_of, state, W); };
  uint32_t s = W.start_bits ? (uint32_t)rfl((int)W.start_bits[row]) : f2u(0.0f);
  int ring_rc = 0;
  auto row_start = [&]() -> uint32_t {
    if (!W.ring || W.rank == 0) return W.start_bits ? (uint32_t)rfl((int)W.start_bits[row]) : f2u(0.0f);
    const RingLayout RL{W.world};
    uint32_t v = 0u;
    ring_rc = ring_wait(W, RL.start(row), v, kRingWalkTicks);
    if (ring_rc == 2 && lane == 0) ring_raise_abort(W, 0x100u | (uint32_t)row);
    return (uint32_t)rfl((int)v);
  };
  uint32_t n_run = 0, n_runfail = 0, n_recfail = 0, n_tab_nw = 0, n_tab_cross = 0;
  uint32_t n_mail = 0;
  asm volatile("" : "+v"(n_run), "+v"(n_runfail), "+v"(n_recfail), "+v"(n_tab_nw), "+v"(n_tab_cross), "+v"(n_mail));
  unsigned long long ticks_scan = 0, ticks_walk = 0;
  const long long t_enter = trace_clock(W);
  const unsigned long long c_enter = (W.selfcheck & 2) ? (unsigned long long)__builtin_readcyclecounter() : 0ull;
  {
    const int64_t chunk = (int64_t)my_chunk * kChainTiles;
    const long long t_a = stat_clock(W);
    if (threadIdx.x < kChainSegs) {
      s_sufok[threadIdx.x] = 0;
      s_mail[threadIdx.x].req = 0;
      s_mail[threadIdx.x].ack = 0;
    }
    if (threadIdx.x < kTabSlots) s_tab_ord[threadIdx.x] = 0;
    if (threadIdx.x == 0) {
      s_progress = 0;
      s_pre_cnt[0] = s_pre_cnt[1] = 0;
      s_np_ok = 0;
    }
    if (threadIdx.x < 8) s_wk[threadIdx.x] = 0ull;
    static_assert(kWalker != 0, "wave 0 fetches the loop state: it must not be the walker");
    if (fuse_update && threadIdx.x < 18) {
      if (threadIdx.x < 16) s_pose[threadIdx.x] = state->trans[threadIdx.x];
      else s_pose_n[threadIdx.x - 16] = threadIdx.x == 16 ? state->iter : state->num_iteration;
    }
    TileRec R;
    R.key = -2;
    R.in = R.out = 0u;
    R.cons = 0;
    R.s = summary_identity();
    bool head = true, tail = true, valid = false;
    {
      const int64_t tile = chunk + threadIdx.x;
      valid = tile < W.ntiles;
      if (valid) R = W.recs[row * W.ntiles + tile];
      if ((W.selfcheck & 2) && last_chunk && walker) {
        const unsigned long long tt = clock_after((uint32_t)R.key);
        if (lane == 0) s_wk[4] = tt;
      }
      rec_put(s_rec, threadIdx.x, R);
      const int32_t key_prev = lane_prev(R.key, R.key), key_next = lane_next(R.key, R.key);
      const int alone = stands_alone(R) ? 1 : 0, alone_prev = lane_prev(alone, 0), alone_next = lane_next(alone, 0);
      head = lane == 0 || R.key < 0 || R.key != key_prev || alone || alone_prev;
      tail = lane == 63 || R.key < 0 || R.key != key_next || alone || alone_next;
      const unsigned long long tails = __ballot(tail && valid);
      if (tail && valid) {
        const unsigned long long below = tails & ((1ull << lane) - 1ull);
        const int idx = wave * 64 + __popcll(below);
        s_tail[idx] = (int16_t)threadIdx.x;
        s_head[idx] = (int16_t)(wave * 64 + (below ? 64 - __builtin_clzll(below) : 0));
      }
      if (lane == 0) s_count[wave] = __popcll(tails);
      const unsigned long long aux = __ballot(valid && (R.cons >> 8) != 0);
      if (lane == 0) {
        s_auxcnt[wave] = __popcll(aux);
        s_auxmask[wave][0] = (uint32_t)aux;
        s_auxmask[wave][1] = (uint32_t)(aux >> 32);
      }
    }
    if (done) return;
    __syncthreads();
    int naux = 0;
    {
      int base = 0;
      for (int w = 0; w < kChainSegs; w++) {
        const int c = s_auxcnt[w];
        base += w < wave ? c : 0;
        naux += c;
      }
      const bool has = valid && (R.cons >> 8) != 0;
      const unsigned long long aux = __ballot(has);
      const int ord = base + __popcll(aux & ((1ull << lane) - 1ull));
      s_auxord[threadIdx.x] = has ? (int16_t)ord : (int16_t)-1;
      if (has) s_auxlist[ord] = (int16_t)threadIdx.x;
    }
    __syncthreads();
    if (!walker) {
      auto scan_forwards = [&](int seg, TileRec P, bool is_head) {
        int fp = is_head ? 1 : 0;
        auto step = [&](const TileRec &X, int xf, bool takes) {
          if (takes && !fp) {
            P = compose_rec(X, P);
            fp = xf;
          }
        };
        step(dpp_rec<0x111, 0xf>(P), dpp_int<0x111, 0xf>(fp), (lane & 15) >= 1);
        step(dpp_rec<0x112, 0xf>(P), dpp_int<0x112, 0xf>(fp), (lane & 15) >= 2);
        step(dpp_rec<0x114, 0xf>(P), dpp_int<0x114, 0xf>(fp), (lane & 15) >= 4);
        step(dpp_rec<0x118, 0xf>(P), dpp_int<0x118, 0xf>(fp), (lane & 15) >= 8);
        step(dpp_rec<0x142, 0xa>(P), dpp_int<0x142, 0xa>(fp), (lane & 16) != 0);
        step(dpp_rec<0x143, 0xc>(P), dpp_int<0x143, 0xc>(fp), lane >= 32);
        rec_put(s_pre, seg * 64 + lane, P);
        lds_fence_wave();
        if (lane == 0) __hip_atomic_fetch_add(&s_pre_cnt[seg >> 2], 1, __ATOMIC_RELEASE, __HIP_MEMORY_SCOPE_WORKGROUP);
      };
      const bool have_cand = !(W.selfcheck & 4);
      uint32_t cand_out[kCand / kLanes];
#pragma unroll
      for (int j = 0; j < kCand / kLanes; j++) cand_out[j] = 0x7fc00000u;
      if (wave < naux && have_cand) {
        const int slot = (s_rec[3][s_auxlist[wave]] >> 8) - 1;
        const uint32_t *tab = W.cand + (size_t)slot * kCand + lane;
#pragma unroll
        for (int j = 0; j < kCand / kLanes; j++) cand_out[j] = tab[j * kLanes];
      }
      scan_forwards(wave, R, head);
      if (wave < naux) {
#pragma unroll
        for (int j = 0; j < kCand / kLanes; j++) s_tab[wave][j * kLanes + lane] = cand_out[j];
        lds_fence_wave();
        if (lane == 0) lds_put(&s_tab_ord[wave], wave + 1);
      }
      const bool second_early = wave + kHelpers < naux;
      if (second_early) {
#pragma unroll
        for (int j = 0; j < kCand / kLanes; j++) cand_out[j] = 0x7fc00000u;
        if (have_cand) {
          const int slot = (s_rec[3][s_auxlist[wave + kHelpers]] >> 8) - 1;
          const uint32_t *tab = W.cand + (size_t)slot * kCand + lane;
#pragma unroll
          for (int j = 0; j < kCand / kLanes; j++) cand_out[j] = tab[j * kLanes];
        }
      }
      if (wave == kWalker - 4) {
        const TileRec Ro = rec_get(s_rec, kWalker * 64 + lane);
        const int32_t kp = lane_prev(Ro.key, Ro.key);
        const int ao = stands_alone(Ro) ? 1 : 0, ao_prev = lane_prev(ao, 0);
        scan_forwards(kWalker, Ro, lane == 0 || Ro.key < 0 || Ro.key != kp || ao || ao_prev);
      }
      auto scan_backwards = [&](int seg, TileRec Q, bool is_tail) {
        int fq = is_tail ? 1 : 0;
        auto behind = [&](const TileRec &Y, int yf, bool takes) {
          if (takes && !fq) {
            Q = compose_rec(Q, Y);
            fq = yf;
          }
        };
        behind(dpp_rec<0x101, 0xf>(Q), dpp_int<0x101, 0xf>(fq), (lane & 15) + 1 < 16);
        behind(dpp_rec<0x102, 0xf>(Q), dpp_int<0x102, 0xf>(fq), (lane & 15) + 2 < 16);
        behind(dpp_rec<0x104, 0xf>(Q), dpp_int<0x104, 0xf>(fq), (lane & 15) + 4 < 16);
        behind(dpp_rec<0x108, 0xf>(Q), dpp_int<0x108, 0xf>(fq), (lane & 15) + 8 < 16);
        {
          const int src = (lane & ~15) + 16;
          const TileRec Y = shfl_rec(Q, src);
          const int yf = __shfl(fq, src);
          behind(Y, yf, !(lane & 16));
        }
        {
          const TileRec Y = shfl_rec(Q, 32);
          const int yf = __shfl(fq, 32);
          behind(Y, yf, lane < 32);
        }
        rec_put(s_suf, seg * 64 + lane, Q);
        lds_fence_wave();
        if (lane == 0) lds_put(&s_sufok[seg], 1);
      };
      constexpr int kQuiet = kWalker - 4;
      if (wave != kQuiet) scan_backwards(wave, R, tail);
      if (second_early) {
#pragma unroll
        for (int j = 0; j < kCand / kLanes; j++) s_tab[wave + kHelpers][j * kLanes + lane] = cand_out[j];
        lds_fence_wave();
        if (lane == 0) lds_put(&s_tab_ord[wave + kHelpers], wave + kHelpers + 1);
      }
      if (wave == 0 || wave == 2) {
        const int seg = wave == 0 ? kWalker : kQuiet;
        const TileRec Ro = rec_get(s_rec, seg * 64 + lane);
        const int32_t kn = lane_next(Ro.key, Ro.key);
        const int ao = stands_alone(Ro) ? 1 : 0, ao_next = lane_next(ao, 0);
        scan_backwards(seg, Ro, lane == 63 || Ro.key < 0 || Ro.key != kn || ao || ao_next);
      }
      if (row == 0 && wave == 1 && last_chunk) {
        unsigned long long v = 0ull;
        for (int64_t t = lane; t < W.ntiles; t += kLanes) v += W.tile_pairs[t];
#pragma unroll
        for (int o = 32; o > 0; o >>= 1) v += __shfl_xor(v, o);
        if (lane == 0) {
          s_np = v;
          lds_put(&s_np_ok, 1);
        }
      }
      int k = wave;
      while (k < naux) {
        const int cur_tile = s_auxlist[k];
        const int32_t cur_key = s_rec[0][cur_tile];
        const int slot = (s_rec[3][cur_tile] >> 8) - 1;
        const int cur_kind = cur_key >= 0 ? JOB_CROSSING : JOB_NOWINDOW;
        const LeafAux A = W.aux[(size_t)slot * kLanes + lane];
        float t[kLeaf];
        load_leaf_quads(W.aux_terms + (size_t)slot * (kTile / 4), lane, t);
        const uint32_t g0 = (uint32_t)s_rec[1][cur_tile];
        if (k != wave && k + kHelpers < naux) {
          const int next_slot = (s_rec[3][s_auxlist[k + kHelpers]] >> 8) - 1;
#pragma unroll
          for (int j = 0; j < kCand / kLanes; j++) cand_out[j] = 0x7fc00000u;
          if (have_cand) {
            const uint32_t *tab = W.cand + (size_t)next_slot * kCand + lane;
#pragma unroll
            for (int j = 0; j < kCand / kLanes; j++) cand_out[j] = tab[j * kLanes];
          }
#pragma unroll
          for (int j = 0; j < kCand / kLanes; j++) s_tab[(k + kHelpers) % kTabSlots][j * kLanes + lane] = cand_out[j];
          lds_fence_wave();
          if (lane == 0) lds_put(&s_tab_ord[(k + kHelpers) % kTabSlots], k + kHelpers + 1);
        }
#pragma unroll
        for (int j = 0; j < kCand / kLanes; j++) cand_out[j] = s_tab[k % kTabSlots][j * kLanes + lane];
        bool serve = false;
        while (true) {
          if (lds_get(&s_mail[wave].req) == k + 1) {
            serve = true;
            break;
          }
// ... 482 lines not shown
                    if (T.key >= 0) n_tab_cross++;
                    else n_tab_nw++;
                  }
                }
              }
              if (from_table) {
              } else if (ord >= 0) {
                n_mail += 1u << why;
                ChainMail *M = &s_mail[ord % kHelpers];
                if (lane == 0) {
                  __hip_atomic_store(&M->s_in, s, __ATOMIC_RELAXED, __HIP_MEMORY_SCOPE_WORKGROUP);
                  lds_put(&M->req, ord + 1);
                }
                const long long t_m = stat_clock(W);
                while (lds_get(&M->ack) != ord + 1) {
                }
                if ((W.selfcheck & 8) && lane == 0) { s_wk[1] += (unsigned long long)(stat_clock(W) - t_m); s_wk[2] += 1ull; }
                s = (uint32_t)rfl((int)__hip_atomic_load(&M->s_out, __ATOMIC_RELAXED, __HIP_MEMORY_SCOPE_WORKGROUP));
              } else {
                const long long t_begin = stat_clock(W);
                recompute_tile_to_lds(term_src(), row, chunk + f, lane, s_tile);
                LeafAux none;
                int serial, tried, applied;
                s = resolve_staged<false>(s, 0, -1, none, lane, s_tile, nullptr, serial, tried, applied);
                __builtin_amdgcn_wave_barrier();
                if (lane == 0) resolve_stats(W, 0, serial, tried, applied, stat_clock(W) - t_begin);
              }
            }
            selfcheck<kCheck>(W, term_src, row, s_in, s, chunk + f, chunk + f + 1, 2, lane, s_tile);
            f++;
            if (f > e) break;
            const long long t_s = stat_clock(W);
            while (lds_get(&s_sufok[f >> 6]) == 0) {
            }
            if ((W.selfcheck & 8) && lane == 0) s_wk[3] += (unsigned long long)(stat_clock(W) - t_s);
            const TileRec Sf = load_rec_uniform(s_suf, f);
            const uint32_t s_in2 = s;
            if ((Sf.key >= 0 && apply(s, Sf.key, Sf.s)) || apply_point(s, Sf)) {
              selfcheck<kCheck>(W, term_src, row, s_in2, s, chunk + f, chunk + e + 1, 3, lane, s_tile);
              break;
            }
          }
          if (lane == 0) lds_put(&s_progress, e + 1);
          if ((W.selfcheck & 8) && lane == 0) s_wk[0] += (unsigned long long)(stat_clock(W) - t_fail);
        }
        if (W.selfcheck & 8) {
          const unsigned long long tt = clock_after(s);
          if (lane == 0) s_wk[5] += tt - (unsigned long long)t_j0;
        }
      }
      if (!last_chunk && lane == 0 && ring_rc == 0)
        __hip_atomic_store(W.chunk_state + ((size_t)row * W.nchunks + my_chunk + 1) * 16, (unsigned long long)W.epoch << 32 | s,
                           __ATOMIC_RELAXED, __HIP_MEMORY_SCOPE_AGENT);
      if (last_chunk && W.ring && ring_rc == 0 && lane == 0) {
        const RingLayout RL{W.world};
        if (W.rank < W.world - 1) ring_put(ring_inbox(W, W.rank + 1) + RL.start(row), s, W.ring_epoch);
        else
          for (int k = 0; k < W.world - 1; k++) ring_put(ring_inbox(W, k) + RL.final(row), s, W.ring_epoch);
      }
      if (lane == 0) {
        lds_put(&s_progress, 1 << 30);
        ticks_scan += (unsigned long long)(t_b - t_a);
        ticks_walk += (unsigned long long)(stat_clock(W) - t_b);
        s_stat[0] = n_run; s_stat[1] = n_runfail; s_stat[2] = n_recfail; s_stat[3] = n_tab_nw; s_stat[4] = n_tab_cross; s_stat[5] = n_mail;
        s_stat_ticks[0] = ticks_scan; s_stat_ticks[1] = ticks_walk;
      }
    }
    __syncthreads();
  }
  if (wave == 0 && lane == 0) {
    const unsigned long long scan_ticks = s_stat_ticks[0], walk_ticks = s_stat_ticks[1];
    atomicAdd(&W.dbg[0], (unsigned long long)s_stat[0]);
    atomicAdd(&W.dbg[1], (unsigned long long)s_stat[1]);
    atomicAdd(&W.dbg[4], (unsigned long long)s_stat[2]);
    atomicAdd(&W.dbg[8], scan_ticks);
    atomicAdd(&W.dbg[9], walk_ticks);
    atomicMax(&W.dbg[14 + 32], walk_ticks);
    atomicAdd(&W.dbg[27 + row], walk_ticks);
    if (W.selfcheck & 8) {
      for (int k = 0; k < 6; k++) atomicAdd(&W.dbg[36 + k], s_wk[k]);
      atomicAdd(&W.dbg[60], s_wk[6]);
      if (last_chunk) atomicAdd(&W.dbg[61], s_wk[6]);
    } else {
      atomicAdd(&W.dbg[36 + row], (unsigned long long)s_stat[2]);
    }
    atomicAdd(&W.dbg[24], (unsigned long long)s_stat[3]);
    atomicAdd(&W.dbg[25], (unsigned long long)s_stat[3]);
    atomicAdd(&W.dbg[45], (unsigned long long)s_stat[4]);
    if (W.selfcheck & 8) {
      atomicAdd(&W.dbg[42], (unsigned long long)(s_stat[5] & 0xffu));
      atomicAdd(&W.dbg[43], (unsigned long long)((s_stat[5] >> 8) & 0xffu));
      atomicAdd(&W.dbg[44], (unsigned long long)((s_stat[5] >> 16) & 0xffu));
    }
  }
  if (!last_chunk) return;
  if (walker && lane == 0 && (W.selfcheck & 2)) {
    W.stamps[row * 16 + 11] = (unsigned long long)t_enter;
    W.stamps[row * 16 + 10] = (unsigned long long)__builtin_readcyclecounter() - c_enter;
    W.stamps[row * 16 + 12] = s_wk[4];
    W.stamps[row * 16 + 13] = s_wk[5];
    W.stamps[row * 16 + 14] = (unsigned long long)n_run | ((unsigned long long)n_runfail << 16) |
                              ((unsigned long long)n_recfail << 32) | ((unsigned long long)(n_tab_nw + n_tab_cross) << 48);
    W.stamps[row * 16 + 15] = (unsigned long long)trace_clock(W);
  }
  if (W.ring && walker) {
    const RingLayout RL{W.world};
    unsigned long long pairs = 0ull;
    if (row == 0) {
      while (lds_get(&s_np_ok) == 0) __builtin_amdgcn_s_sleep(1);
      pairs = s_np;
      if (W.rank > 0 && ring_rc == 0) {
        uint32_t lo = 0u, hi = 0u;
        ring_rc = ring_wait(W, RL.start_pairs(), lo, kRingWalkTicks);
        if (ring_rc == 0) ring_rc = ring_wait(W, RL.start_pairs() + 1, hi, kRingWalkTicks);
        pairs += (unsigned long long)hi << 32 | lo;
      }
      if (ring_rc == 0 && lane == 0) {
        if (W.rank < W.world - 1) {
          unsigned long long *dst = ring_inbox(W, W.rank + 1) + RL.start_pairs();
          ring_put(dst, (uint32_t)pairs, W.ring_epoch);
          ring_put(dst + 1, (uint32_t)(pairs >> 32), W.ring_epoch);
        } else {
          for (int k = 0; k < W.world - 1; k++) {
            unsigned long long *dst = ring_inbox(W, k) + RL.final_pairs();
            ring_put(dst, (uint32_t)pairs, W.ring_epoch);
            ring_put(dst + 1, (uint32_t)(pairs >> 32), W.ring_epoch);
          }
        }
      }
    }
    if (W.rank < W.world - 1 && ring_rc == 0) {
      uint32_t v = 0u;
      ring_rc = ring_wait(W, RL.final(row), v, kRingWalkTicks);
      s = (uint32_t)rfl((int)v);
      if (row == 0 && ring_rc == 0) {
        uint32_t lo = 0u, hi = 0u;
        ring_rc = ring_wait(W, RL.final_pairs(), lo, kRingWalkTicks);
        if (ring_rc == 0) ring_rc = ring_wait(W, RL.final_pairs() + 1, hi, kRingWalkTicks);
        pairs = (unsigned long long)hi << 32 | lo;
      }
    }
    if (ring_rc != 0) {
      if (lane == 0) {
        if (ring_rc == 2) ring_raise_abort(W, 0x200u | (uint32_t)row);
        state->status = PCGX_E_RCCL;
        state->done = 1;
      }
      return;
    }
    if (row == 0 && lane == 0) __hip_atomic_store(&sums10[S_PAIRS], (double)pairs, __ATOMIC_RELAXED, __HIP_MEMORY_SCOPE_AGENT);
  } else if (row == 0 && walker && lane == 0) {
    while (lds_get(&s_np_ok) == 0) __builtin_amdgcn_s_sleep(1);
    if (!W.hop_out) __hip_atomic_store(&sums10[S_PAIRS], (double)s_np, __ATOMIC_RELAXED, __HIP_MEMORY_SCOPE_AGENT);
  }
  if (walker) {
    unsigned ticket = 0u;
    if (lane == 0) {
      const int slot = row == 0 ? S_VALUE : (row <= 6 ? S_G0 + row - 1 : (row == 7 ? S_DIST_RMS : S_WEIGHT));
      if (W.hop_out) W.hop_out[row] = (double)s;
      else __hip_atomic_store(&sums10[slot], (double)u2f(s), __ATOMIC_RELAXED, __HIP_MEMORY_SCOPE_AGENT);
      if (W.hop_out) __threadfence();
      else asm volatile("s_waitcnt vmcnt(0)" ::: "memory");
      ticket = atomicAdd(W.done_rows, 1u);
    }
    ticket = (unsigned)rfl((int)ticket);
    if (ticket == (unsigned)W.nrows - 1u) {
      static_assert(kAuxShards == kLanes, "a shard's counter per lane");
      W.aux_count[lane * 32] = 0u;
      if (W.exchange)
        for (int64_t k = lane, n = (W.ntiles + 31) / 32, m = n + (n + 31) / 32; k < m; k += kLanes) W.tile_arrived[32 * k] = 0u;
      if (lane == 0) *W.done_rows = 0u;
      if (!W.hop_out && lane == 0) {
        double sums[S_COUNT];
        for (int k = 0; k < S_COUNT; k++) sums[k] = __hip_atomic_load(&sums10[k], __ATOMIC_RELAXED, __HIP_MEMORY_SCOPE_AGENT);
        const unsigned long long np = (unsigned long long)sums[S_PAIRS];
        if (W.nrows < kStrictRows) {
          sums[S_WEIGHT] = (double)(np < (1ull << 24) ? np : (1ull << 24));
          sums10[S_WEIGHT] = sums[S_WEIGHT];
        }
        const long long t_u0 = trace_clock(W);
        if (fuse_update) icp_update_step(state, sums, kp, s_pose, s_pose_n);
        if (W.selfcheck & 2) {
          __threadfence();
          W.stamps[kStrictRows * 16 + 14] = (unsigned long long)t_u0;
          W.stamps[kStrictRows * 16 + 15] = (unsigned long long)trace_clock(W);
        }
      }
    }
  }
}

struct StrictBuffers {
  StrictWork w = {};
  StrictKnobs knobs;
  StrictLayout layout;
  void *block = nullptr;
  double *shard = nullptr;
  int shard_world = 0;
  bool shard_ring = false;
  std::vector<void *> retired;
  uint8_t *at(int region) const { return (uint8_t *)block + layout.region[region].offset; }
};

constexpr StrictFacts kFacts;
static_assert(kFacts.rows == kStrictRows && kFacts.tile == kTile && kFacts.lanes == kLanes && kFacts.chain_tiles == kChainTiles &&
                  kFacts.aux_shards == kAuxShards && kFacts.cand == kCand && kFacts.repair_block == kRepairBlock &&
                  kFacts.repair_min_tiles == kRepairMinTiles && kFacts.job_roles == kJobRoles && kFacts.tile_rec == sizeof(TileRec) &&
                  kFacts.leaf_aux == sizeof(LeafAux) && kFacts.job_desc == sizeof(JobDesc),
              "strict_plan.h plans with the kernels' constants");

static StrictKnobs strict_knobs() {
  const auto num = [](const char *name, int absent) {
    const char *e = getenv(name);
    return e ? atoi(e) : absent;
  };
  static const bool repair_on = num("PCGX_STRICT_REPAIR", 1) != 0, spec_on = num("PCGX_STRICT_SPEC", 1) != 0;
  StrictKnobs k;
  k.spec_depth = num("PCGX_STRICT_SPEC_DEPTH", 4);
  k.selfcheck = (getenv("PCGX_STRICT_SELFCHECK") ? 1 : 0) | (getenv("PCGX_STRICT_TRACE") ? 2 : 0) |
                (getenv("PCGX_STRICT_NOSPEC") ? 4 : 0) | (getenv("PCGX_STRICT_CLOCKS") ? 8 : 0) | (getenv("PCGX_TEST_SPEC_MISS") ? 16 : 0);
  k.exchange = num("PCGX_STRICT_EXCHANGE", 1) != 0 ? 1 : 0;
  k.slots_per_shard = num("PCGX_STRICT_SLOTS_PER_SHARD", -1);
  k.repair_on = repair_on;
  k.spec_on = spec_on;
  return k;
}

static hipError_t zero_runs(const StrictBuffers *b, const StrictLayout::Run *runs, int n, hipStream_t st) {
  hipError_t e = hipSuccess;
  for (int i = 0; i < n && e == hipSuccess; i++) {
    const StrictLayout::Span s = b->layout.span(runs[i]);
    e = hipMemsetAsync((uint8_t *)b->block + s.offset, 0, s.bytes, st);
  }
  return e;
}

pcgx_status strict_create(int64_t nt, const float *tx, const float *ty, const float *tz, const uint32_t *pos_of,
                          StrictBuffers **out, hipStream_t st) {
  StrictBuffers *b = new StrictBuffers();
  b->knobs = strict_knobs();
  b->layout = plan_strict_layout(nt, b->knobs, kFacts);
  const StrictLayout &L = b->layout;
  hipError_t e = dev_cache_alloc(&b->block, L.total);
  if (e != hipSuccess) {
    const size_t total = L.total;
    delete b;
    return fail(PCGX_E_OOM, "strict sums: allocation of %zu bytes failed: %s", total, hipGetErrorString(e));
  }
  StrictWork &W = b->w;
  W.nt = nt;
  W.first_exact = 1;
  W.ring_guess_ticks = kRingGuessTicks;
  W.world = 1;
  W.ntiles = L.ntiles;
  W.ntiles_pad = L.ntiles_pad;
  W.nchunks = L.nchunks;
  W.naux = L.naux;
  W.nrows = kStrictRows;
  W.spec_depth = b->knobs.spec_depth;
  W.selfcheck = b->knobs.selfcheck;
  W.exchange = b->knobs.exchange;
  W.tile_sum = (double *)b->at(kRegTileSum);
  W.tile_err = (double *)b->at(kRegTileErr);
  W.tile_pub = (double *)b->at(kRegTilePub);
  W.tile_arrived = (unsigned int *)b->at(kRegTileArrived);
  W.tile_pairs = (uint32_t *)b->at(kRegTilePairs);
  W.recs = (TileRec *)b->at(kRegRecs);
  W.aux = (LeafAux *)b->at(kRegAux);
  W.aux_terms = (float4 *)b->at(kRegAuxTerms);
  W.jobs = (JobDesc *)b->at(kRegJobs);
  W.cand = (uint32_t *)b->at(kRegCand);
  W.xyz_caller = (const float *)b->at(kRegXyzCaller);
  W.done_rows = (unsigned int *)(b->at(kRegCounters) + kDoneRowsAt);
  W.aux_count = (unsigned int *)(b->at(kRegCounters) + kAuxCountAt);
  W.dbg = (unsigned long long *)b->at(kRegDbg);
  W.stamps = (unsigned long long *)b->at(kRegStamps);
  W.chunk_state = (unsigned long long *)b->at(kRegChunkState);
  e = zero_runs(b, L.zero_create, 3, st);
  if (e == hipSuccess && nt > 0) {
    hipLaunchKernelGGL(strict_xyz_caller_kernel, dim3((unsigned)((nt + 255) / 256)), dim3(256), 0, st, tx, ty, tz, pos_of, nt,
                       const_cast<float *>(W.xyz_caller));
    e = hipGetLastError();
  }
  if (e != hipSuccess) {
    dev_cache_free(b->block);
    delete b;
    return fail(PCGX_E_HIP, "strict sums: hipMemsetAsync failed: %s", hipGetErrorString(e));
  }
  *out = b;
  return PCGX_OK;
}

void strict_destroy(StrictBuffers *b) {
  if (!b) return;
  dev_cache_free(b->shard);
  for (void *p : b->retired) dev_cache_free(p);
  dev_cache_free(b->block);
  delete b;
}

const StrictWork *strict_work(StrictBuffers *b, const IcpKernelParams &kp) {
  b->w.weight_fn = kp.weight_fn;
  b->w.weight_a = kp.weight_a;
  b->w.nrows = kp.weight_fn == PCGX_WEIGHT_ONE ? kStrictRows - 1 : kStrictRows;
  return &b->w;
}
static const StrictWork &next_epoch(StrictBuffers *b) {
  if (++b->w.epoch == 0u) b->w.epoch = 1u;
  return b->w;
}

struct StepArgs {
  const float4 *match;
  const uint32_t *pos_of;
  IcpState *state;
  double *sums10;
  const IcpKernelParams &kp;
  hipStream_t st;
  const CertifiedTerms *certify = nullptr;
};
static StrictStep step_of(StrictBuffers *b, const IcpKernelParams &kp) {
  const StrictWork &W = *strict_work(b, kp);
  StrictStep s;
  s.ntiles = W.ntiles;
  s.nchunks = W.nchunks;
  s.naux = W.naux;
  s.nrows = W.nrows;
  return s;
}
static void launch_tilesum(const StrictWork &W, const StepArgs &a) {
  hipLaunchKernelGGL(strict_tilesum_kernel, dim3((unsigned)W.ntiles), dim3(kTileSumBlock), 0, a.st, a.match, a.pos_of,
                     (const IcpState *)a.state, W);
}
enum : unsigned { kStageSummary = 1, kStageJobs = 2, kStageChain = 4 };
static pcgx_status enqueue_stages(unsigned stages, const StrictLaunches &L, const StrictWork &W, const StepArgs &a) {
  if (!L.live) return PCGX_OK;
  const IcpState *state = a.state;
  if ((stages & kStageSummary) && L.summary != kSumNone) {
    ProfScope prof(PCGX_PROF_STRICT_SUM, a.st);
    const dim3 grid((unsigned)W.ntiles), block(kSumBlock);
    if (L.summary == kSumPlain)
      hipLaunchKernelGGL(strict_sum_kernel<false>, grid, block, 0, a.st, a.match, a.pos_of, state, W);
    else if (L.summary == kSumExchange)
      hipLaunchKernelGGL(strict_sum_kernel<true>, grid, block, 0, a.st, a.match, a.pos_of, state, W);
    else if (L.summary == kSumRing)
      hipLaunchKernelGGL((strict_sum_kernel<true, true>), grid, block, 0, a.st, a.match, a.pos_of, state, W);
    else if (L.summary == kSumCertified)
      hipLaunchKernelGGL((strict_sum_kernel<true, false, true>), grid, block, 0, a.st, a.match, a.pos_of, state, W, *a.certify);
    else
      return fail(PCGX_E_INVALID, "strict sums: the certified terms need the exchange and the pairs in the caller's order");
  }
  if (stages & kStageJobs) {
    ProfScope prof(PCGX_PROF_STRICT_JOB, a.st);
    if (L.repair_grid)
      hipLaunchKernelGGL(strict_repair_kernel, dim3(L.repair_grid), dim3(kRepairBlock), 0, a.st, a.match, a.pos_of, state, W);
    if (L.jobs_grid) hipLaunchKernelGGL(strict_job_kernel, dim3(L.jobs_grid), dim3(kJobBlock), 0, a.st, state, W);
  }
  if ((stages & kStageChain) && L.chain != kChainNone) {
    ProfScope prof(PCGX_PROF_STRICT_CHAIN, a.st);
    const dim3 grid(L.chain_grid), block(kChainBlock);
    if (L.chain == kChainCheck)
      hipLaunchKernelGGL((strict_chain_kernel<true, false>), grid, block, 0, a.st, a.match, a.pos_of, a.state, W, a.sums10, a.kp, L.fuse_update);
    else if (L.chain == kChainSpec)
      hipLaunchKernelGGL((strict_chain_kernel<false, true>), grid, block, 0, a.st, a.match, a.pos_of, a.state, W, a.sums10, a.kp, L.fuse_update);
    else
      hipLaunchKernelGGL((strict_chain_kernel<false, false>), grid, block, 0, a.st, a.match, a.pos_of, a.state, W, a.sums10, a.kp, L.fuse_update);
  }
  return PCGX_OK;
}

pcgx_status strict_enqueue(StrictBuffers *b, const float4 *match, const uint32_t *pos_of, IcpState *state,
                           double *sums10, const IcpKernelParams &kp, bool fuse_update, bool have_tile_sums, bool first_iter,
                           hipStream_t st, const CertifiedTerms *certify) {
  StrictStep s = step_of(b, kp);
  s.have_tile_sums = have_tile_sums;
  s.first_iter = first_iter;
  s.certify = certify != nullptr;
  s.caller_order = pos_of == nullptr;
  s.fuse_update = fuse_update;
  const StrictLaunches L = plan_strict_launches(kOneGpu, s, b->knobs, kFacts);
  const StrictWork &W = next_epoch(b);
  const StepArgs a{match, pos_of, state, sums10, kp, st, certify};
  if (L.tilesum) {
    ProfScope prof(PCGX_PROF_STRICT_TERMS, st);
    launch_tilesum(W, a);
  }
  PCGX_TRY(enqueue_stages(kStageSummary | kStageJobs | kStageChain, L, W, a));
  PCGX_HIP_TRY(hipGetLastError());
  return PCGX_OK;
}

__global__ __launch_bounds__(64) void strict_row_totals_kernel(const double *__restrict__ per_tile, const uint32_t *__restrict__ tile_pairs,
                                                               int64_t ntiles, int nrows, const IcpState *__restrict__ state,
                                                               double *__restrict__ slot ) {
  const int row = blockIdx.x, lane = threadIdx.x;
  if (state->done) return;
  if (row < nrows) {
    double v = 0.0;
    for (int64_t t = lane; t < ntiles; t += 64) v += per_tile[(int64_t)row * ntiles + t];
    v = wave_allsum_f64(v);
    if (lane == 0) slot[row] = v;
  } else if (row == kStrictRows && tile_pairs) {
    double v = 0.0;
    for (int64_t t = lane; t < ntiles; t += 64) v += (double)tile_pairs[t];
    v = wave_allsum_f64(v);
    if (lane == 0) slot[kStrictRows] = v;
  }
}
__global__ void strict_base_kernel(const double *__restrict__ slots, int rank, int world, double *__restrict__ out) {
  const int r = threadIdx.x;
  if (r < kStrictRows) {
    double v = 0.0;
    for (int k = 0; k < rank; k++) v += slots[k * 16 + r];
    out[r] = v;
  } else if (r == kStrictRows) {
    double v = 0.0;
    for (int k = 0; k < world; k++) v += slots[k * 16 + r];
    out[r] = v;
  }
}
__global__ void strict_hop_kernel(const double *__restrict__ hop, uint32_t *__restrict__ start_bits) {
  if (threadIdx.x < kStrictRows) start_bits[threadIdx.x] = (uint32_t)hop[threadIdx.x];
}
__global__ void strict_zero_kernel(double *__restrict__ p, int n, double last) {
  if ((int)threadIdx.x < n) p[threadIdx.x] = ((int)threadIdx.x == n - 1) ? last : 0.0;
}
__global__ void strict_finish_kernel(const uint32_t *__restrict__ end_bits, const double *__restrict__ err_base ,
                                     const double *__restrict__ failed, int nrows, IcpState *__restrict__ state,
                                     double *__restrict__ sums10, IcpKernelParams kp) {
  if (threadIdx.x != 0 || blockIdx.x != 0) return;
  if (state->done) return;
  if (*failed != 0.0) {
    state->status = PCGX_E_RCCL;
    state->done = 1;
    return;
  }
  double sums[S_COUNT];
  for (int row = 0; row < nrows; row++) {
    const int slot = row == 0 ? S_VALUE : (row <= 6 ? S_G0 + row - 1 : (row == 7 ? S_DIST_RMS : S_WEIGHT));
    sums[slot] = (double)u2f(end_bits[row]);
  }
  const double np = err_base[kStrictRows];
  sums[S_PAIRS] = np;
  if (nrows < kStrictRows) sums[S_WEIGHT] = np < 16777216.0 ? np : 16777216.0;
  for (int k = 0; k < S_COUNT; k++) sums10[k] = sums[k];
  icp_update_step(state, sums, kp);
}

static pcgx_status ensure_shard(StrictBuffers *b, int world, bool want_ring, hipStream_t st) {
  const ShardPlan p = plan_shard(b->shard != nullptr, b->shard_world, b->shard_ring, world, want_ring);
  if (p.allocate) {
    if (b->shard) b->retired.push_back(b->shard);
    b->shard = nullptr;
    if (dev_cache_alloc((void **)&b->shard, p.bytes) != hipSuccess)
      return fail(PCGX_E_OOM, "strict sums over ranks: no memory for the exchange");
    b->shard_world = world;
  }
  if (p.zero) PCGX_HIP_TRY(hipMemsetAsync(b->shard, 0, p.bytes, st));
  b->shard_ring = p.ring;
  return PCGX_OK;
}

pcgx_status strict_enqueue_sharded(StrictBuffers *b, const float4 *match, const uint32_t *pos_of, IcpState *state, double *sums10,
                                   const IcpKernelParams &kp, pcgx_comm *c, int rank, int world, bool local_failed, hipStream_t st) {
  PCGX_TRY(ensure_shard(b, world, false, st));
  double *slots = b->shard, *row_base = slots + (size_t)world * 16, *err_base = row_base + 16, *hop = row_base + 32;
  uint32_t *start_bits = reinterpret_cast<uint32_t *>(hop + 16);
  StrictStep s = step_of(b, kp);
  s.rank = rank;
  s.world = world;
  s.local_failed = local_failed;
  const StrictLaunches L = plan_strict_launches(kCollective, s, b->knobs, kFacts);
  const StepArgs a{match, pos_of, state, sums10, kp, st};
  StrictWork W = next_epoch(b);
  W.row_base = row_base;
  W.err_base = err_base;
  W.start_bits = start_bits;
  W.hop_out = hop;
  W.first_exact = rank == 0 ? 1 : 0;
  auto exchange = [&](double *d_buf, int count, int flag_at) -> pcgx_status {
    if (local_failed) {
      static const double one = 1.0;
      PCGX_HIP_TRY(hipMemcpyAsync(d_buf + flag_at, &one, sizeof one, hipMemcpyHostToDevice, st));
    }
    return pcgx_comm_allreduce_f64(c, d_buf, count, st);
  };
  const int nslots = world * 16;
  PCGX_HIP_TRY(hipMemsetAsync(slots, 0, (size_t)nslots * sizeof(double), st));
  if (L.live) {
    ProfScope prof(PCGX_PROF_STRICT_TERMS, st);
    if (L.tilesum) launch_tilesum(W, a);
    hipLaunchKernelGGL(strict_row_totals_kernel, dim3(kStrictRows), dim3(64), 0, st, (const double *)W.tile_sum,
                       (const uint32_t *)nullptr, W.ntiles, W.nrows, (const IcpState *)state, slots + (size_t)rank * 16);
  }
  PCGX_TRY(exchange(slots, nslots, rank * 16 + 10));
  if (L.live) hipLaunchKernelGGL(strict_base_kernel, dim3(1), dim3(64), 0, st, (const double *)slots, rank, world, row_base);
  PCGX_TRY(enqueue_stages(kStageSummary, L, W, a));
  PCGX_HIP_TRY(hipMemsetAsync(slots, 0, (size_t)nslots * sizeof(double), st));
  if (L.live)
    hipLaunchKernelGGL(strict_row_totals_kernel, dim3(kStrictRows + 1), dim3(64), 0, st, (const double *)W.tile_err,
                       (const uint32_t *)W.tile_pairs, W.ntiles, W.nrows, (const IcpState *)state, slots + (size_t)rank * 16);
  PCGX_TRY(exchange(slots, nslots, rank * 16 + 10));
  hipLaunchKernelGGL(strict_base_kernel, dim3(1), dim3(64), 0, st, (const double *)slots, rank, world, err_base);
  PCGX_TRY(enqueue_stages(kStageJobs, L, W, a));
  hipLaunchKernelGGL(strict_zero_kernel, dim3(1), dim3(64), 0, st, reinterpret_cast<double *>(start_bits), 8, 0.0);
  for (int k = 0; k < world; k++) {
    hipLaunchKernelGGL(strict_zero_kernel, dim3(1), dim3(64), 0, st, hop, 16, 0.0);
    if (k == rank) PCGX_TRY(enqueue_stages(kStageChain, L, W, a));
    PCGX_TRY(exchange(hop, 16, 10));
    hipLaunchKernelGGL(strict_hop_kernel, dim3(1), dim3(64), 0, st, (const double *)hop, start_bits);
  }
  hipLaunchKernelGGL(strict_finish_kernel, dim3(1), dim3(64), 0, st, (const uint32_t *)start_bits, (const double *)err_base,
                     (const double *)(hop + 10), W.nrows, state, sums10, kp);
  PCGX_HIP_TRY(hipGetLastError());
  return PCGX_OK;
}

__global__ __launch_bounds__(64) void strict_ring_err_kernel(const IcpState *__restrict__ state, StrictWork W) {
  const int lane = threadIdx.x, b = blockIdx.x;
  if (state->done) return;
  const RingLayout RL{W.world};
  if (b < kStrictRows) {
    if (b >= W.nrows || W.rank >= W.world - 1) return;
    double v = 0.0;
    for (int64_t t = lane; t < W.ntiles; t += 64) v += W.tile_err[(int64_t)b * W.ntiles + t];
    v = wave_allsum_f64(v);
    if (lane < W.world - 1 - W.rank)
      ring_put_f64(ring_inbox(W, W.rank + 1 + lane) + RL.err_tot(W.rank, b), v, W.ring_epoch);
    return;
  }
  double acc = 0.0;
  for (int k0 = 0; k0 < W.rank; k0 += 7) {
    const int k = k0 + lane / kStrictRows, row = lane % kStrictRows;
// ... 159 lines not shown
```

pcgol_amd/csrc/strict_plan.h:

```cpp
#pragma once
#include <cstddef>
#include <cstdint>

namespace pcgx {

struct StrictFacts {
  int32_t rows = 9;
  int32_t tile = 2048;
  int32_t lanes = 64;
  int32_t chain_tiles = 512;
  int32_t aux_shards = 64;
  int32_t cand = 768;
  int32_t repair_block = 512;
  int64_t repair_min_tiles = 1024;
  int32_t job_roles = 3;
  size_t tile_rec = 64, leaf_aux = 96, job_desc = 16;
};

struct StrictKnobs {
  int32_t spec_depth = 4;
  int32_t selfcheck = 0;
  int32_t exchange = 1;
  int32_t slots_per_shard = -1;
  bool repair_on = true;
  bool spec_on = true;
};

enum StrictRegion : int32_t {
  kRegTileSum, kRegTileErr, kRegTilePub, kRegTileArrived, kRegTilePairs, kRegRecs, kRegAux, kRegAuxTerms, kRegJobs,
  kRegCand, kRegXyzCaller, kRegCounters, kRegDbg, kRegStamps, kRegChunkState,
  kStrictRegions
};
constexpr size_t kDoneRowsAt = 12, kAuxCountAt = 256;

struct StrictLayout {
  struct Span {
    size_t offset, bytes;
  };
  struct Run {
    int32_t first, last;
  };
  int64_t ntiles = 1, ntiles_pad = 128;
  int32_t nchunks = 1, naux = 0;
  Span region[kStrictRegions] = {};
  size_t total = 0;
  Run zero_create[3] = {{kRegCounters, kRegDbg}, {kRegTileArrived, kRegTileArrived}, {kRegChunkState, kRegChunkState}};
  Run zero_reset[2] = {{kRegCounters, kRegCounters}, {kRegTileArrived, kRegTileArrived}};
  Span span(Run r) const { return {region[r.first].offset, region[r.last].offset + region[r.last].bytes - region[r.first].offset}; }
};

inline StrictLayout plan_strict_layout(int64_t nt, const StrictKnobs &k, const StrictFacts &f = StrictFacts()) {
  StrictLayout L;
  L.ntiles = nt > 0 ? (nt + f.tile - 1) / f.tile : 1;
  L.ntiles_pad = (L.ntiles + 127) & ~(int64_t)127;
  L.nchunks = (int32_t)((L.ntiles + f.chain_tiles - 1) / f.chain_tiles);
  L.naux = (int32_t)(f.aux_shards * ((f.rows * L.ntiles / 4 + f.aux_shards - 1) / f.aux_shards + 4));
  if (k.slots_per_shard >= 0 && (int64_t)k.slots_per_shard * f.aux_shards < L.naux) L.naux = k.slots_per_shard * f.aux_shards;
  const size_t nt1 = (size_t)L.ntiles, na = (size_t)L.naux;
  const int64_t n_groups = (L.ntiles + 31) / 32;
  const auto set = [&L](StrictRegion r, size_t bytes) { L.region[r].bytes = bytes; };
  set(kRegTileSum, (size_t)f.rows * nt1 * sizeof(double));
  set(kRegTileErr, (size_t)f.rows * nt1 * sizeof(double));
  set(kRegTilePub, (size_t)L.ntiles_pad * 16 * sizeof(double));
  set(kRegTileArrived, (size_t)(n_groups + (n_groups + 31) / 32) * 128);
  set(kRegTilePairs, nt1 * sizeof(uint32_t));
  set(kRegRecs, (size_t)f.rows * nt1 * f.tile_rec);
  set(kRegAux, na * f.lanes * f.leaf_aux);
  set(kRegAuxTerms, na * f.tile * sizeof(float));
  set(kRegJobs, na * f.job_desc);
  set(kRegCand, na * f.cand * sizeof(uint32_t));
  set(kRegXyzCaller, (size_t)(nt ? nt : 1) * 12 + 64);
  set(kRegCounters, kAuxCountAt + (size_t)f.aux_shards * 128);
  set(kRegDbg, 64 * sizeof(unsigned long long));
  set(kRegStamps, nt1 * 16 * sizeof(unsigned long long));
  set(kRegChunkState, (size_t)f.rows * L.nchunks * 16 * sizeof(unsigned long long));
  for (int r = 0; r < kStrictRegions; r++) {
    L.region[r].offset = L.total;
    L.region[r].bytes = (L.region[r].bytes + 255) & ~(size_t)255;
    L.total += L.region[r].bytes;
  }
  return L;
}

enum StrictForm : int32_t { kOneGpu, kCollective, kRing };
enum StrictSummary : int32_t {
  kSumNone,
  kSumPlain,
  kSumExchange,
  kSumRing,
  kSumCertified,
  kSumCertifyError
};
enum StrictChain : int32_t {
  kChainNone,
  kChainCheck,
  kChainSpec,
  kChainPlain
};

struct StrictStep {
  int64_t ntiles = 1;
  int32_t nchunks = 1, naux = 0, nrows = 9;
  int32_t rank = 0, world = 1;
  bool have_tile_sums = false;
  bool first_iter = false;
  bool certify = false;
  bool caller_order = false;
  bool fuse_update = false;
  bool local_failed = false;
};

struct StrictLaunches {
  bool live = true;
  bool tilesum = false;
  int32_t summary = kSumNone;
  int32_t exchange = 1;
  bool bases_behind_summary = false;
  uint32_t ring_err_grid = 0;
  uint32_t repair_grid = 0, jobs_grid = 0;
  int32_t chain = kChainNone;
  uint32_t chain_grid = 0;
  int32_t fuse_update = 0;
};

inline StrictLaunches plan_strict_launches(StrictForm form, const StrictStep &s, const StrictKnobs &k,
                                           const StrictFacts &f = StrictFacts()) {
  StrictLaunches L;
  L.exchange = form == kRing ? 1 : k.exchange;
  if (form != kOneGpu && s.local_failed) {
    L.live = false;
    return L;
  }
  if (form == kOneGpu) {
    L.tilesum = !s.have_tile_sums && !k.exchange;
    L.summary = s.certify ? (k.exchange && s.caller_order ? kSumCertified : kSumCertifyError) : (k.exchange ? kSumExchange : kSumPlain);
    if (L.summary == kSumCertifyError) return L;
  } else if (form == kCollective) {
    L.tilesum = true;
    L.summary = kSumPlain;
  } else {
    L.summary = kSumRing;
    L.ring_err_grid = s.world > 1 ? (uint32_t)(f.rows + (s.rank > 0 ? 1 : 0)) : 0u;
    L.bases_behind_summary = s.rank > 0;
  }
  if (form != kCollective && s.first_iter && s.naux > 0 && s.ntiles >= f.repair_min_tiles && k.repair_on)
    L.repair_grid = (uint32_t)(s.nrows * ((s.ntiles + f.repair_block - 1) / f.repair_block));
  if (s.naux > 0) L.jobs_grid = (uint32_t)f.job_roles * (uint32_t)s.naux;
  const bool waits = form == kRing || s.nchunks > 1;
  const int64_t walks_ahead = (int64_t)(form == kRing ? s.rank : 0) * s.nchunks + s.nchunks - 1;
  L.chain = (k.selfcheck & 1) ? kChainCheck : (waits && k.spec_on && walks_ahead >= k.spec_depth ? kChainSpec : kChainPlain);
  L.chain_grid = (uint32_t)(s.nrows * s.nchunks);
  L.fuse_update = form == kOneGpu ? (s.fuse_update ? 1 : 0) : (form == kRing ? 1 : 0);
  return L;
}

struct ShardPlan {
  bool allocate;
  bool zero;
  size_t bytes;
  bool ring;
};
inline ShardPlan plan_shard(bool have_block, int block_world, bool block_ring, int world, bool want_ring) {
  const bool allocate = !have_block || block_world != world;
  return {allocate, want_ring && (allocate || !block_ring), (size_t)(world + 4) * 16 * sizeof(double), want_ring};
}

}
```

pcgol_amd/csrc/strict_terms.h:

```cpp
#pragma once
#include "pcgx_internal.h"
#include "strict_sum.h"

namespace pcgx {
using namespace ss;

constexpr int kStrictRows = 9;


template <int kCtrl, int kRowMask>
__device__ __forceinline__ double dpp_f64(double old, double v) {
  constexpr bool kZeroFill = kRowMask == 0xf;
  const unsigned long long o = (unsigned long long)__double_as_longlong(old), x = (unsigned long long)__double_as_longlong(v);
  const uint32_t lo = (uint32_t)__builtin_amdgcn_update_dpp((int)(uint32_t)o, (int)(uint32_t)x, kCtrl, kRowMask, 0xf, kZeroFill);
  const uint32_t hi = (uint32_t)__builtin_amdgcn_update_dpp((int)(uint32_t)(o >> 32), (int)(uint32_t)(x >> 32), kCtrl, kRowMask, 0xf, kZeroFill);
  return __longlong_as_double((long long)((unsigned long long)hi << 32 | lo));
}
__device__ __forceinline__ double lane_f64(double v, int src) {
  const unsigned long long x = (unsigned long long)__double_as_longlong(v);
  const uint32_t lo = (uint32_t)__builtin_amdgcn_readlane((int)(uint32_t)x, src), hi = (uint32_t)__builtin_amdgcn_readlane((int)(uint32_t)(x >> 32), src);
  return __longlong_as_double((long long)((unsigned long long)hi << 32 | lo));
}
__device__ __forceinline__ double wave_allsum_f64(double v) {
  v += dpp_f64<0x111, 0xf>(0.0, v);
// ... 62 lines not shown
  const uint32_t *start_bits;
  double *hop_out;
  int32_t first_exact;
  unsigned long long *chunk_state;
  int32_t nchunks;
  uint32_t epoch;
  unsigned long long *ring;
  int32_t ring_words;
  unsigned long long *const *ring_tab;
  unsigned long long *ring_mine;
  int32_t rank, world;
  uint32_t ring_epoch;
  long long ring_guess_ticks;
  double *ring_base;
  unsigned int *ring_flag;
  int32_t spec_depth;
  int32_t selfcheck;
};

struct CertifiedTerms {
  GridView grid;
  float max_dist_sq;
  float4 *match_caller;
  float4 *match;
  float *match_cert;
  const uint32_t *pos_of;
  int32_t test_force_walk;
  int32_t test_force_grid_walk;
};

struct RingLayout {
  int world;
  __host__ __device__ int row_tot(int k, int row) const { return (k * kStrictRows + row) * 2; }
  __host__ __device__ int err_tot(int k, int row) const { return world * 2 * kStrictRows + (k * kStrictRows + row) * 2; }
  __host__ __device__ int start(int row) const { return world * 4 * kStrictRows + row; }
  __host__ __device__ int start_pairs() const { return world * 4 * kStrictRows + kStrictRows; }
  __host__ __device__ int final(int row) const { return world * 4 * kStrictRows + 16 + row; }
  __host__ __device__ int final_pairs() const { return world * 4 * kStrictRows + 16 + kStrictRows; }
  __host__ __device__ int abort() const { return world * 4 * kStrictRows + 32; }
  __host__ __device__ int words() const { return (world * 4 * kStrictRows + 33 + 15) & ~15; }
};
constexpr int kRingTagStepBits = 12;
constexpr long long kRingGuessTicks = 200000;
constexpr long long kRingGuessTicksApart = 20000000;
constexpr long long kRingWalkTicks = 1000000000;

#if defined(__HIPCC__)
__device__ __forceinline__ void ring_put(unsigned long long *w, uint32_t payload, uint32_t epoch) {
  __hip_atomic_store(w, (unsigned long long)epoch << 32 | payload, __ATOMIC_RELAXED, __HIP_MEMORY_SCOPE_SYSTEM);
}
__device__ __forceinline__ void ring_put_f64(unsigned long long *w, double v, uint32_t epoch) {
  const unsigned long long x = (unsigned long long)__double_as_longlong(v);
  ring_put(w, (uint32_t)x, epoch);
  ring_put(w + 1, (uint32_t)(x >> 32), epoch);
}
__device__ __forceinline__ bool ring_peek(const unsigned long long *w, uint32_t epoch, uint32_t &payload) {
  const unsigned long long v = __hip_atomic_load(w, __ATOMIC_RELAXED, __HIP_MEMORY_SCOPE_SYSTEM);
  payload = (uint32_t)v;
  return (uint32_t)(v >> 32) == epoch;
}
__device__ __forceinline__ bool ring_aborted(const StrictWork &W) {
  const RingLayout RL{W.world};
  const unsigned long long v = __hip_atomic_load(W.ring + (size_t)W.rank * W.ring_words + RL.abort(), __ATOMIC_RELAXED, __HIP_MEMORY_SCOPE_SYSTEM);
  const uint32_t tag = (uint32_t)(v >> 32);
  return tag != 0u && tag >> kRingTagStepBits == W.ring_epoch >> kRingTagStepBits && tag <= W.ring_epoch;
}
__device__ __forceinline__ unsigned long long *ring_inbox(const StrictWork &W, int k) { return W.ring_tab[k]; }
__device__ __forceinline__ int ring_wait(const StrictWork &W, int off, uint32_t &payload, long long max_ticks) {
  const unsigned long long *p = W.ring_mine + off;
  long long t_first = 0;
  for (int spins = 0;; spins++) {
    if (ring_peek(p, W.ring_epoch, payload)) return 0;
    if ((spins & 15) == 15) {
      if (ring_aborted(W)) return 1;
      const long long now = (long long)wall_clock64();
      if (t_first == 0) t_first = now;
      if (now - t_first > max_ticks) return 2;
    }
    __builtin_amdgcn_s_sleep(8);
  }
}
__device__ __forceinline__ int ring_wait_f64(const StrictWork &W, int off, double &v, long long max_ticks) {
  uint32_t lo = 0u, hi = 0u;
  int rc = ring_wait(W, off, lo, max_ticks);
  if (rc == 0) rc = ring_wait(W, off + 1, hi, max_ticks);
  v = __longlong_as_double((long long)((unsigned long long)hi << 32 | lo));
  return rc;
}
__device__ __forceinline__ void ring_raise_abort(const StrictWork &W, uint32_t reason) {
  const RingLayout RL{W.world};
  for (int k = 0; k < W.world; k++) ring_put(W.ring + (size_t)k * W.ring_words + RL.abort(), reason, W.ring_epoch);
}
#endif

struct TermSrc {
  const float4 *match;
  const uint32_t *pos_of;
  const float *xyz;
  int64_t nt;
  float m[16];
  bool project;
  int32_t weight_fn;
  float weight_a;
  const float *raw;
};

__device__ __forceinline__ TermSrc make_term_src(const float4 *match, const uint32_t *pos_of, const IcpState *state,
                                                 const StrictWork &W) {
  TermSrc S;
  S.match = match;
  S.pos_of = pos_of;
  S.xyz = W.xyz_caller;
  S.nt = W.nt;
#pragma unroll
  for (int k = 0; k < 16; k++) S.m[k] = state->trans[k];
  S.project = state->iter > 0;
  S.weight_fn = W.weight_fn;
  S.weight_a = W.weight_a;
  S.raw = W.raw_terms;
  return S;
}

__device__ __forceinline__ bool pair_terms(const TermSrc &S, float x0, float y0, float z0, const float4 &b, float *t ) {
#pragma unroll
  for (int k = 0; k < kStrictRows; k++) t[k] = -0.0f;
  if (!(b.w >= 0.0f)) return false;
  if (S.raw) {
    const int64_t i = (int64_t)__float_as_int(x0);
#pragma unroll
    for (int k = 0; k < kStrictRows; k++) t[k] = S.raw[(int64_t)k * S.nt + i];
    return true;
  }
  if (S.project) {
    float px, py, pz;
    mat4_transform(S.m, x0, y0, z0, px, py, pz);
    x0 = px; y0 = py; z0 = pz;
  }
  const float x1 = b.x, y1 = b.y, z1 = b.z;
  const float ddx = x1 - x0, ddy = y1 - y0, ddz = z1 - z0;
  const float dsq = (ddx * ddx + ddy * ddy) + ddz * ddz;
  const float w = eval_weight_fn(S.weight_fn, S.weight_a, dsq);
  t[0] = w * dsq;
  t[1] = w * (x0 - x1);
  t[2] = w * (y0 - y1);
  t[3] = w * (z0 - z1);
  t[4] = w * (z0 * y1 - y0 * z1);
  t[5] = w * (x0 * z1 - z0 * x1);
  t[6] = w * (y0 * x1 - x0 * y1);
  t[7] = w * norm_sq3(x0, y0, z0);
  t[8] = w;
  return true;
}

__device__ __forceinline__ void load_quad(const TermSrc &S, int64_t i0, float4 *bp, float *tx, float *ty, float *tz) {
  if (S.raw) {
#pragma unroll
    for (int c = 0; c < 4; c++) {
      const int64_t i = i0 + c;
      bp[c] = make_float4(0.0f, 0.0f, 0.0f, i < S.nt ? 0.0f : -1.0f);
      tx[c] = __int_as_float((int)i);
      ty[c] = tz[c] = 0.0f;
    }
    return;
  }
  if (i0 + 3 < S.nt) {
    if (S.pos_of) {
      const uint4 p = *reinterpret_cast<const uint4 *>(S.pos_of + i0);
      bp[0] = S.match[p.x]; bp[1] = S.match[p.y]; bp[2] = S.match[p.z]; bp[3] = S.match[p.w];
    } else {
#pragma unroll
      for (int c = 0; c < 4; c++) bp[c] = S.match[i0 + c];
    }
    const float4 *x4 = reinterpret_cast<const float4 *>(S.xyz + 3 * i0);
    const float4 a = x4[0], b = x4[1], d = x4[2];
    tx[0] = a.x; ty[0] = a.y; tz[0] = a.z;
    tx[1] = a.w; ty[1] = b.x; tz[1] = b.y;
    tx[2] = b.z; ty[2] = b.w; tz[2] = d.x;
    tx[3] = d.y; ty[3] = d.z; tz[3] = d.w;
    return;
  }
#pragma unroll
  for (int c = 0; c < 4; c++) {
    const int64_t i = i0 + c;
    bp[c] = make_float4(0.0f, 0.0f, 0.0f, -1.0f);
    tx[c] = ty[c] = tz[c] = 0.0f;
    if (i < S.nt) {
      bp[c] = S.pos_of ? S.match[S.pos_of[i]] : S.match[i];
      tx[c] = S.xyz[3 * i];
      ty[c] = S.xyz[3 * i + 1];
      tz[c] = S.xyz[3 * i + 2];
    }
  }
}

template <int kThreads>
__device__ __forceinline__ void tile_sums_block(const TermSrc &S, const StrictWork &W, int64_t tile, double (*s_part)[kStrictRows]) {
  constexpr int kQuads = kTile / 4 / kThreads;
  static_assert(kQuads >= 1 && kQuads * kThreads * 4 == kTile, "the block covers the tile");
  double acc[kStrictRows];
#pragma unroll
  for (int k = 0; k < kStrictRows; k++) acc[k] = 0.0;
  float4 bp[kQuads][4];
  float tx[kQuads][4], ty[kQuads][4], tz[kQuads][4];
#pragma unroll
  for (int h = 0; h < kQuads; h++)
    load_quad(S, tile * kTile + 4 * (int64_t)(h * kThreads + threadIdx.x), bp[h], tx[h], ty[h], tz[h]);
#pragma unroll
  for (int h = 0; h < kQuads; h++) {
    float t[4][kStrictRows];
#pragma unroll
    for (int c = 0; c < 4; c++) pair_terms(S, tx[h][c], ty[h][c], tz[h][c], bp[h][c], t[c]);
#pragma unroll
    for (int k = 0; k < kStrictRows; k++) acc[k] += (((double)t[0][k] + (double)t[1][k]) + (double)t[2][k]) + (double)t[3][k];
  }
  const int lane = threadIdx.x & 63, wave = threadIdx.x >> 6;
#pragma unroll
  for (int k = 0; k < kStrictRows; k++) {
    const double v = wave_allsum_f64(acc[k]);
    if (lane == 0) s_part[wave][k] = v;
  }
  __syncthreads();
  if ((int)threadIdx.x < W.nrows) {
    double v = 0.0;
    for (int w = 0; w < kThreads / 64; w++) v += s_part[w][threadIdx.x];
    W.tile_sum[threadIdx.x * W.ntiles + tile] = v;
  }
  __syncthreads();
}

}
```

Before: 15230.

## Defer ICP pose update into next certified summary kernel

On certified steps, the pose update that used to run at the end of the strict chain kernel (a serial tail behind the last row's ticket) is deferred. Each block of the next iteration's certified summary kernel recomputes it while its point loads are in flight, and the last tile writes the updated state back. A flush path launches a standalone update kernel whenever the deferred update cannot be folded in: non-certified steps, settle, or the last iteration. This shortens the critical path at the end of each iteration, at the cost of redundant per-block update math and added state-handoff complexity.

```diff
diff --git a/pcgol_amd/csrc/icp.hip b/pcgol_amd/csrc/icp.hip
--- a/pcgol_amd/csrc/icp.hip
+++ b/pcgol_amd/csrc/icp.hip
@@ -650,6 +650,7 @@
   bool spec_walk = true;
   bool spec_pending = false;
   hipStream_t spec_stream = nullptr;
+  bool update_pending = false;
   hipStream_t used[4] = {nullptr, nullptr, nullptr, nullptr};
   int n_used = 0;
   void touch(hipStream_t st) {
@@ -680,6 +681,7 @@
 };
 
 static pcgx_status settle(pcgx_icp_session *s, hipStream_t st);
+static pcgx_status flush_update(pcgx_icp_session *s, hipStream_t st);
 static int icp_knob(const char *name, int def, int lo, int hi);
 
 static pcgx_status enter(pcgx_icp_session *s, void *stream, hipStream_t *st) {
@@ -768,6 +770,7 @@
   hipLaunchKernelGGL(icp_reset_kernel, dim3(blocks), dim3(zero_words ? 256 : 64), 0, st, s->d_state, z);
   PCGX_HIP_TRY(hipGetLastError());
   s->host_iter = 0;
+  s->update_pending = false;
   if (s->shard_failed || s->steps_sharded > 0) {
     PCGX_TRY(strict_reset(s->strict_buf, st));
     s->shard_failed = false;
@@ -815,7 +818,7 @@
   if (!s) return fail(PCGX_E_INVALID, "pcgx_icp_session_set_strict: NULL session");
   if (on && s->plane) return fail(PCGX_E_INVALID, "pcgx_icp_session_set_strict: point-to-plane sessions have no reference sums to reproduce");
   if (on < 0 || on > 2) return fail(PCGX_E_INVALID, "pcgx_icp_session_set_strict: mode must be 0, 1 or 2");
-  if (s->spec_pending) PCGX_TRY(settle(s, s->spec_stream));
+  if (s->spec_pending || s->update_pending) PCGX_TRY(settle(s, s->spec_stream));
   s->strict = on;
   s->strict_explicit = on != 0;
   return PCGX_OK;
@@ -1092,9 +1095,11 @@
     k.cert_on = icp_knob("PCGX_ICP_CERT", 1, 0, 1) != 0;
     k.spec_on = icp_knob("PCGX_ICP_SPEC_WALK", 1, 0, 1) != 0;
     k.fused_from = icp_knob("PCGX_ICP_FUSED_FROM", 2, 0, 1 << 30);
+    k.defer_on = icp_knob("PCGX_ICP_DEFER_UPDATE", 1, 0, 1) != 0;
     k.test_force_walk = icp_knob("PCGX_TEST_ICP_FORCE_WALK", 0, 0, 1 << 30);
     k.test_fused_search = icp_knob("PCGX_TEST_ICP_FUSED_SEARCH", 0, 0, 1 << 30);
     k.test_fused_grid_walk = icp_knob("PCGX_TEST_ICP_FUSED_GRID_WALK", 0, 0, 1 << 30);
+    k.test_fused_grid_walk_from = icp_knob("PCGX_TEST_ICP_FUSED_GRID_WALK_FROM", 0, 0, 1 << 30);
     return k;
   }();
   return knobs;
@@ -1143,6 +1148,7 @@
   f.host_iter = s->host_iter;
   f.may_speculate = may_speculate;
   f.grid = s->grid;
+  f.max_iteration = s->max_iteration;
   *plan = plan_step(f, step_knobs());
   s->caller_order_fresh = plan->next_caller_had_pairs;
   if (plan->no_walk) {
@@ -1253,11 +1259,19 @@
       C.match_cert = s->d_match_cert;
       C.pos_of = s->d_pos_of;
       C.test_force_walk = step_knobs().test_fused_search;
-      C.test_force_grid_walk = step_knobs().test_fused_grid_walk;
+      C.test_force_grid_walk = s->host_iter > step_knobs().test_fused_grid_walk_from ? step_knobs().test_fused_grid_walk : 0;
     }
     const StrictPairs pairs = strict_pairs(s, p.sums_caller);
-    PCGX_TRY(strict_enqueue(s->strict_buf, pairs.match, pairs.pos_of, s->d_state, s->d_sums, s->kp, kFuseUpdate,
-                            p.have_tile_sums, p.first_iter, st, p.certify ? &C : nullptr));
+    const bool defer = kFuseUpdate && p.defer_update, apply = s->update_pending;
+    bool deferred = false;
+    s->update_pending = false;
+    PCGX_TRY(strict_enqueue(s->strict_buf, pairs.match, pairs.pos_of, s->d_state, s->d_sums, s->kp, kFuseUpdate && !defer,
+                            p.have_tile_sums, p.first_iter, st, p.certify ? &C : nullptr, apply, defer, &deferred));
+    s->update_pending = deferred;
+    if (defer && !deferred) {
+      s->update_pending = true;
+      PCGX_TRY(flush_update(s, st));
+    }
   } else if (s->strict) {
     if (!s->d_terms) {
       s->nt_pad = (s->nt + 63) & ~(int64_t)63;
@@ -1288,11 +1302,21 @@
 static pcgx_status enqueue_step(pcgx_icp_session *s, hipStream_t st, bool may_speculate) {
   StepPlan plan;
   PCGX_TRY(decide_step(s, st, may_speculate, &plan));
+  if (!plan.certify) PCGX_TRY(flush_update(s, st));
   PCGX_TRY(enqueue_corr(s, st, plan));
   return enqueue_sums<kFuseUpdate>(s, st, plan);
 }
 
+static pcgx_status flush_update(pcgx_icp_session *s, hipStream_t st) {
+  if (!s->update_pending) return PCGX_OK;
+  s->update_pending = false;
+  hipLaunchKernelGGL(icp_update_kernel<false>, dim3(1), dim3(64), 0, st, s->d_state, (const double *)s->d_sums, s->kp);
+  PCGX_HIP_TRY(hipGetLastError());
+  return PCGX_OK;
+}
+
 static pcgx_status settle(pcgx_icp_session *s, hipStream_t st) {
+  PCGX_TRY(flush_update(s, st));
   if (!s->spec_pending) return PCGX_OK;
   s->spec_pending = false;
   IcpState h;
diff --git a/pcgol_amd/csrc/icp_step_plan.h b/pcgol_amd/csrc/icp_step_plan.h
--- a/pcgol_amd/csrc/icp_step_plan.h
+++ b/pcgol_amd/csrc/icp_step_plan.h
@@ -18,6 +18,7 @@
   int32_t host_iter = 0;
   bool may_speculate = false;
   int32_t grid = 1;
+  int32_t max_iteration = 0;
 };
 
 struct StepKnobs {
@@ -27,9 +28,11 @@
   bool cert_on = true;
   bool spec_on = true;
   int32_t fused_from = 2;
+  bool defer_on = true;
   int32_t test_force_walk = 0;
   int32_t test_fused_search = 0;
   int32_t test_fused_grid_walk = 0;
+  int32_t test_fused_grid_walk_from = 0;
 };
 
 enum CorrForm : int32_t {
@@ -53,6 +56,7 @@
   bool have_tile_sums = false;
   bool first_iter = false;
   bool next_caller_had_pairs = false;
+  bool defer_update = false;
 };
 
 inline StepPlan plan_step(const StepFacts &f, const StepKnobs &k) {
@@ -75,6 +79,7 @@
   p.certify = p.no_walk && k.fused_from > 0 && f.host_iter >= k.fused_from && p.cert && f.caller_had_pairs && caller &&
               f.exchange;
   p.corr = p.certify ? kCorrNone : p.no_walk ? kCorrGrid : grid ? kCorrGridWalk : kCorrWalk;
+  p.defer_update = p.certify && k.defer_on && f.host_iter + 1 < f.max_iteration;
   return p;
 }
 
diff --git a/pcgol_amd/csrc/pcgx_internal.h b/pcgol_amd/csrc/pcgx_internal.h
--- a/pcgol_amd/csrc/pcgx_internal.h
+++ b/pcgol_amd/csrc/pcgx_internal.h
@@ -309,7 +309,8 @@
 const StrictWork *strict_work(StrictBuffers *b, const IcpKernelParams &kp);
 pcgx_status strict_enqueue(StrictBuffers *b, const float4 *match, const uint32_t *pos_of, IcpState *state,
                            double *sums10, const IcpKernelParams &kp, bool fuse_update, bool have_tile_sums, bool first_iter,
-                           hipStream_t st, const struct CertifiedTerms *certify = nullptr);
+                           hipStream_t st, const struct CertifiedTerms *certify = nullptr, bool apply_pending = false,
+                           bool defer_update = false, bool *deferred = nullptr);
 pcgx_status strict_read_debug(StrictBuffers *b, unsigned long long out[64], hipStream_t st);
 pcgx_status strict_check_enqueue(const float *d_xyz, int64_t nt, int64_t nt_pad, const float4 *match, const uint32_t *pos_of,
                                  IcpState *state, const IcpKernelParams &kp, float *d_terms, unsigned long long *d_valid,
diff --git a/pcgol_amd/csrc/strict.hip b/pcgol_amd/csrc/strict.hip
--- a/pcgol_amd/csrc/strict.hip
+++ b/pcgol_amd/csrc/strict.hip
@@ -426,17 +426,73 @@
   return n;
 }
 
-template <bool kExchange, bool kSharded = false, bool kCertify = false>
+constexpr int kUpdWords = 30, kUpdIter = 16, kUpdNumIter = 17, kUpdDone = 18, kUpdStatus = 19, kUpdEv = 20, kUpdMask = 30, kUpdNowDone = 31;
+static_assert(offsetof(IcpState, iter) == 4 * kUpdIter && offsetof(IcpState, num_iteration) == 4 * kUpdNumIter &&
+                  offsetof(IcpState, done) == 4 * kUpdDone && offsetof(IcpState, status) == 4 * kUpdStatus &&
+                  offsetof(IcpState, ev) == 4 * kUpdEv && sizeof(Evaluated) == 40 && offsetof(Evaluated, num_pairs) == 32 &&
+                  offsetof(IcpState, hessian) == 4 * kUpdWords,
+              "the pending update's record is the loop state's first words");
+__device__ __forceinline__ void pending_update(const double *__restrict__ sums10, const float *pose, int32_t iter, int32_t num_iteration,
+                                               int nrows, const IcpKernelParams &kp, uint32_t *out ) {
+  double sums[S_COUNT];
+#pragma unroll
+  for (int k = 0; k < S_COUNT; k++) sums[k] = sums10[k];
+  const unsigned long long np = (unsigned long long)sums[S_PAIRS];
+  if (nrows < kStrictRows) sums[S_WEIGHT] = (double)(np < (1ull << 24) ? np : (1ull << 24));
+  uint32_t mask = 1u << kUpdNumIter;
+  int now_done = 0;
+  out[kUpdNumIter] = (uint32_t)(num_iteration + 1);
+  out[kUpdIter] = (uint32_t)iter;
+  const int64_t npairs = (int64_t)sums[S_PAIRS];
+  out[kUpdEv + 8] = (uint32_t)(unsigned long long)npairs;
+  out[kUpdEv + 9] = (uint32_t)((unsigned long long)npairs >> 32);
+  mask |= 3u << (kUpdEv + 8);
+  if (npairs < (int64_t)kp.min_pairs) {
+#pragma unroll
+    for (int i = 0; i < 16; i++) out[i] = f2u(pose[i]);
+    out[kUpdStatus] = (uint32_t)PCGX_E_NOT_ENOUGH_PAIRS;
+    mask |= 1u << kUpdStatus;
+    now_done = 1;
+  } else {
+    Evaluated ev;
+    finish_evaluate(sums, ev);
+    out[kUpdEv] = f2u(ev.value);
+#pragma unroll
+    for (int i = 0; i < 6; i++) out[kUpdEv + 1 + i] = f2u(ev.gradient[i]);
+    out[kUpdEv + 7] = f2u(ev.dist_rms);
+    Mat4 t;
+#pragma unroll
+    for (int i = 0; i < 16; i++) t.m[i] = pose[i];
+    int32_t it = iter;
+    if (gradient_descent_update(kp.upd, it, ev.gradient, t)) now_done = 1;
+#pragma unroll
+    for (int i = 0; i < 16; i++) out[i] = f2u(t.m[i]);
+    out[kUpdIter] = (uint32_t)it;
+    mask |= 0xffffu | 1u << kUpdIter | 0xffu << kUpdEv;
+  }
+  out[kUpdDone] = 1u;
+  if (now_done) mask |= 1u << kUpdDone;
+  out[kUpdMask] = mask;
+  out[kUpdNowDone] = (uint32_t)now_done;
+}
+__device__ __forceinline__ void pending_update_store(IcpState *state, const uint32_t *upd, int word) {
+  if (word < kUpdWords && ((upd[kUpdMask] >> word) & 1u)) reinterpret_cast<uint32_t *>(state)[word] = upd[word];
+}
+
+template <bool kExchange, bool kSharded = false, bool kCertify = false, bool kUpdate = false>
 __global__ __launch_bounds__(kSumBlock) __attribute__((amdgpu_waves_per_eu(4, 4))) void strict_sum_kernel(
     const float4 *__restrict__ match, const uint32_t *__restrict__ pos_of, const IcpState *__restrict__ state, StrictWork W,
-    CertifiedTerms C = CertifiedTerms()) {
+    CertifiedTerms C = CertifiedTerms(), const double *__restrict__ sums10 = nullptr, IcpKernelParams kp = IcpKernelParams()) {
   __shared__ float4 s_terms[kStrictRows][kTile / 4];
   __shared__ int s_np[kSumWaves];
   __shared__ int s_ns[kCertify ? kSumWaves : 1];
   __shared__ double s_tot[16];
+  __shared__ uint32_t s_upd[kUpdate ? 32 : 1];
   static_assert(!kSharded || kExchange, "the ring form rides on the exchange");
   static_assert(!kCertify || (kExchange && !kSharded), "the certified terms: one GPU, with the exchange");
-  const int done = state->done;
+  static_assert(!kUpdate || kCertify, "the pending update: certified steps only");
+  const int done_found = state->done;
+  int done = done_found;
   const int lane = threadIdx.x & 63, wave = threadIdx.x >> 6;
   const int64_t tile = blockIdx.x;
   const int NR = W.nrows;
@@ -446,12 +502,34 @@
   held.q = -1;
   double P0 = (!kExchange && wave < NR) ? tile_prefix(W.tile_sum, W.ntiles, wave, tile, lane) : 0.0;
   {
-    const TermSrc S = make_term_src(match, pos_of, state, W);
+    TermSrc S = make_term_src(match, pos_of, state, W);
     const int l = threadIdx.x >> 3, v = threadIdx.x & 7;
     float4 bp[4];
     float tx[4], ty[4], tz[4];
     const int64_t i0 = tile * kTile + (int64_t)l * kLeaf + 4 * v;
-    load_quad(S, i0, bp, tx, ty, tz);
+    if (!kUpdate) load_quad(S, i0, bp, tx, ty, tz);
+    if (kUpdate) {
+      auto new_pose = [&]() {
+        if (threadIdx.x == 0) {
+          if (!done_found) pending_update(sums10, S.m, state->iter, state->num_iteration, W.nrows, kp, s_upd);
+          if (W.selfcheck & 2) W.stamps[tile * 16 + 4] = (unsigned long long)trace_clock(W);
+        }
+        __syncthreads();
+      };
+      if ((tile + 1) * kTile <= W.nt && !S.raw) {
+        load_quad_whole(S, i0, bp, tx, ty, tz);
+        new_pose();
+      } else {
+        load_quad(S, i0, bp, tx, ty, tz);
+        new_pose();
+      }
+      if (!done_found) {
+#pragma unroll
+        for (int k = 0; k < 16; k++) S.m[k] = u2f((uint32_t)rfl((int)s_upd[k]));
+        S.project = rfl((int)s_upd[kUpdIter]) > 0;
+        done = rfl((int)s_upd[kUpdNowDone]);
+      }
+    }
     float t[4][kStrictRows];
     int np = 0;
     if (kCertify) {
@@ -490,6 +568,12 @@
   }
   __syncthreads();
   const long long t_p1 = trace_clock(W);
+  if (kUpdate && done && !done_found) {
+    if (threadIdx.x == 0 && atomicAdd(W.done_rows, 1u) == (unsigned)W.ntiles - 1u) {
+      for (int k = 0; k < kUpdWords; k++) pending_update_store(const_cast<IcpState *>(state), s_upd, k);
+      __hip_atomic_store(W.done_rows, 0u, __ATOMIC_RELAXED, __HIP_MEMORY_SCOPE_AGENT);
+    }
+  }
   if (done) return;
   if (threadIdx.x == 0) {
     int np = 0;
@@ -563,6 +647,10 @@
         }
       }
       if (gave_up && lane == 0) atomicAdd(&W.dbg[63], 1ull);
+      if (kUpdate && tile == W.ntiles - 1) {
+        if (!gave_up) pending_update_store(const_cast<IcpState *>(state), s_upd, lane);
+        else if (lane == 0) atomicCAS(&const_cast<IcpState *>(state)->done, 0, 2);
+      }
       if (kSharded && W.rank > 0) {
         if (tile == 0) {
           const RingLayout RL{W.world};
@@ -715,6 +803,7 @@
     certified_store_flush(C, tile, held);
     if (threadIdx.x == 0) {
       if (tile == 0) atomicAdd(&W.dbg[47], 1ull);
+      if (kUpdate && tile == 0) atomicAdd(&W.dbg[46], 1ull);
       int ns = 0;
       for (int w = 0; w < kSumWaves; w++) ns += s_ns[w];
       if (ns > 0) atomicAdd(&W.dbg[59], (unsigned long long)ns);
@@ -1375,7 +1464,7 @@
     }
     if (threadIdx.x < 8) s_wk[threadIdx.x] = 0ull;
     static_assert(kWalker != 0, "wave 0 fetches the loop state: it must not be the walker");
-    if (fuse_update && threadIdx.x < 18) {
+    if (fuse_update == 1 && threadIdx.x < 18) {
       if (threadIdx.x < 16) s_pose[threadIdx.x] = state->trans[threadIdx.x];
       else s_pose_n[threadIdx.x - 16] = threadIdx.x == 16 ? state->iter : state->num_iteration;
     }
@@ -1414,6 +1503,11 @@
       }
     }
     if (done) return;
+    if (fuse_update == kChainEndDeferred && blockIdx.x == 0 && wave == 0) {
+      W.aux_count[lane * 32] = 0u;
+      if (W.exchange)
+        for (int64_t k = lane, n = (W.ntiles + 31) / 32, m = n + (n + 31) / 32; k < m; k += kLanes) W.tile_arrived[32 * k] = 0u;
+    }
     __syncthreads();
     int naux = 0;
     {
@@ -2202,6 +2296,8 @@
   } else if (row == 0 && walker && lane == 0) {
     while (lds_get(&s_np_ok) == 0) __builtin_amdgcn_s_sleep(1);
     if (!W.hop_out) __hip_atomic_store(&sums10[S_PAIRS], (double)s_np, __ATOMIC_RELAXED, __HIP_MEMORY_SCOPE_AGENT);
+    if (fuse_update == kChainEndDeferred && W.nrows < kStrictRows)
+      __hip_atomic_store(&sums10[S_WEIGHT], (double)(s_np < (1ull << 24) ? s_np : (1ull << 24)), __ATOMIC_RELAXED, __HIP_MEMORY_SCOPE_AGENT);
   }
   if (walker) {
     unsigned ticket = 0u;
@@ -2209,10 +2305,13 @@
       const int slot = row == 0 ? S_VALUE : (row <= 6 ? S_G0 + row - 1 : (row == 7 ? S_DIST_RMS : S_WEIGHT));
       if (W.hop_out) W.hop_out[row] = (double)s;
       else __hip_atomic_store(&sums10[slot], (double)u2f(s), __ATOMIC_RELAXED, __HIP_MEMORY_SCOPE_AGENT);
-      if (W.hop_out) __threadfence();
-      else asm volatile("s_waitcnt vmcnt(0)" ::: "memory");
-      ticket = atomicAdd(W.done_rows, 1u);
-    }
+      if (fuse_update != kChainEndDeferred) {
+        if (W.hop_out) __threadfence();
+        else asm volatile("s_waitcnt vmcnt(0)" ::: "memory");
+        ticket = atomicAdd(W.done_rows, 1u);
+      }
+    }
+    if (fuse_update == kChainEndDeferred) return;
     ticket = (unsigned)rfl((int)ticket);
     if (ticket == (unsigned)W.nrows - 1u) {
       static_assert(kAuxShards == kLanes, "a shard's counter per lane");
@@ -2229,7 +2328,7 @@
           sums10[S_WEIGHT] = sums[S_WEIGHT];
         }
         const long long t_u0 = trace_clock(W);
-        if (fuse_update) icp_update_step(state, sums, kp, s_pose, s_pose_n);
+        if (fuse_update == 1) icp_update_step(state, sums, kp, s_pose, s_pose_n);
         if (W.selfcheck & 2) {
           __threadfence();
           W.stamps[kStrictRows * 16 + 14] = (unsigned long long)t_u0;
@@ -2395,8 +2494,11 @@
       hipLaunchKernelGGL(strict_sum_kernel<true>, grid, block, 0, a.st, a.match, a.pos_of, state, W);
     else if (L.summary == kSumRing)
       hipLaunchKernelGGL((strict_sum_kernel<true, true>), grid, block, 0, a.st, a.match, a.pos_of, state, W);
+    else if (L.summary == kSumCertified && !L.apply_pending)
+      hipLaunchKernelGGL((strict_sum_kernel<true, false, true>), grid, block, 0, a.st, a.match, a.pos_of, state, W, *a.certify);
     else if (L.summary == kSumCertified)
-      hipLaunchKernelGGL((strict_sum_kernel<true, false, true>), grid, block, 0, a.st, a.match, a.pos_of, state, W, *a.certify);
+      hipLaunchKernelGGL((strict_sum_kernel<true, false, true, true>), grid, block, 0, a.st, a.match, a.pos_of, state, W, *a.certify,
+                         (const double *)a.sums10, a.kp);
     else
       return fail(PCGX_E_INVALID, "strict sums: the certified terms need the exchange and the pairs in the caller's order");
   }
@@ -2409,26 +2511,32 @@
   if ((stages & kStageChain) && L.chain != kChainNone) {
     ProfScope prof(PCGX_PROF_STRICT_CHAIN, a.st);
     const dim3 grid(L.chain_grid), block(kChainBlock);
+    const int chain_end = L.defer_update ? kChainEndDeferred : L.fuse_update;
     if (L.chain == kChainCheck)
-      hipLaunchKernelGGL((strict_chain_kernel<true, false>), grid, block, 0, a.st, a.match, a.pos_of, a.state, W, a.sums10, a.kp, L.fuse_update);
+      hipLaunchKernelGGL((strict_chain_kernel<true, false>), grid, block, 0, a.st, a.match, a.pos_of, a.state, W, a.sums10, a.kp, chain_end);
     else if (L.chain == kChainSpec)
-      hipLaunchKernelGGL((strict_chain_kernel<false, true>), grid, block, 0, a.st, a.match, a.pos_of, a.state, W, a.sums10, a.kp, L.fuse_update);
+      hipLaunchKernelGGL((strict_chain_kernel<false, true>), grid, block, 0, a.st, a.match, a.pos_of, a.state, W, a.sums10, a.kp, chain_end);
     else
-      hipLaunchKernelGGL((strict_chain_kernel<false, false>), grid, block, 0, a.st, a.match, a.pos_of, a.state, W, a.sums10, a.kp, L.fuse_update);
+      hipLaunchKernelGGL((strict_chain_kernel<false, false>), grid, block, 0, a.st, a.match, a.pos_of, a.state, W, a.sums10, a.kp, chain_end);
   }
   return PCGX_OK;
 }
 
 pcgx_status strict_enqueue(StrictBuffers *b, const float4 *match, const uint32_t *pos_of, IcpState *state,
                            double *sums10, const IcpKernelParams &kp, bool fuse_update, bool have_tile_sums, bool first_iter,
-                           hipStream_t st, const CertifiedTerms *certify) {
+                           hipStream_t st, const CertifiedTerms *certify, bool apply_pending, bool defer_update, bool *deferred) {
   StrictStep s = step_of(b, kp);
+  s.apply_pending = apply_pending;
+  s.defer_update = defer_update;
   s.have_tile_sums = have_tile_sums;
   s.first_iter = first_iter;
   s.certify = certify != nullptr;
   s.caller_order = pos_of == nullptr;
   s.fuse_update = fuse_update;
   const StrictLaunches L = plan_strict_launches(kOneGpu, s, b->knobs, kFacts);
+  if (apply_pending && !L.apply_pending)
+    return fail(PCGX_E_INVALID, "strict sums: a pending pose update can only be applied by the certified summary kernel");
+  if (deferred) *deferred = L.defer_update;
   const StrictWork &W = next_epoch(b);
   const StepArgs a{match, pos_of, state, sums10, kp, st, certify};
   if (L.tilesum) {
diff --git a/pcgol_amd/csrc/strict_plan.h b/pcgol_amd/csrc/strict_plan.h
--- a/pcgol_amd/csrc/strict_plan.h
+++ b/pcgol_amd/csrc/strict_plan.h
@@ -97,6 +97,7 @@
   kChainSpec,
   kChainPlain
 };
+constexpr int32_t kChainEndDeferred = 2;
 
 struct StrictStep {
   int64_t ntiles = 1;
@@ -108,6 +109,8 @@
   bool caller_order = false;
   bool fuse_update = false;
   bool local_failed = false;
+  bool apply_pending = false;
+  bool defer_update = false;
 };
 
 struct StrictLaunches {
@@ -121,6 +124,8 @@
   int32_t chain = kChainNone;
   uint32_t chain_grid = 0;
   int32_t fuse_update = 0;
+  bool defer_update = false;
+  bool apply_pending = false;
 };
 
 inline StrictLaunches plan_strict_launches(StrictForm form, const StrictStep &s, const StrictKnobs &k,
@@ -135,6 +140,7 @@
     L.tilesum = !s.have_tile_sums && !k.exchange;
     L.summary = s.certify ? (k.exchange && s.caller_order ? kSumCertified : kSumCertifyError) : (k.exchange ? kSumExchange : kSumPlain);
     if (L.summary == kSumCertifyError) return L;
+    L.apply_pending = s.apply_pending && L.summary == kSumCertified;
   } else if (form == kCollective) {
     L.tilesum = true;
     L.summary = kSumPlain;
@@ -151,6 +157,7 @@
   L.chain = (k.selfcheck & 1) ? kChainCheck : (waits && k.spec_on && walks_ahead >= k.spec_depth ? kChainSpec : kChainPlain);
   L.chain_grid = (uint32_t)(s.nrows * s.nchunks);
   L.fuse_update = form == kOneGpu ? (s.fuse_update ? 1 : 0) : (form == kRing ? 1 : 0);
+  L.defer_update = form == kOneGpu && s.defer_update && !s.fuse_update && s.certify && L.chain != kChainCheck;
   return L;
 }
 
diff --git a/pcgol_amd/csrc/strict_terms.h b/pcgol_amd/csrc/strict_terms.h
--- a/pcgol_amd/csrc/strict_terms.h
+++ b/pcgol_amd/csrc/strict_terms.h
@@ -238,6 +238,21 @@
   return true;
 }
 
+__device__ __forceinline__ void load_quad_whole(const TermSrc &S, int64_t i0, float4 *bp, float *tx, float *ty, float *tz) {
+  if (S.pos_of) {
+    const uint4 p = *reinterpret_cast<const uint4 *>(S.pos_of + i0);
+    bp[0] = S.match[p.x]; bp[1] = S.match[p.y]; bp[2] = S.match[p.z]; bp[3] = S.match[p.w];
+  } else {
+#pragma unroll
+    for (int c = 0; c < 4; c++) bp[c] = S.match[i0 + c];
+  }
+  const float4 *x4 = reinterpret_cast<const float4 *>(S.xyz + 3 * i0);
+  const float4 a = x4[0], b = x4[1], d = x4[2];
+  tx[0] = a.x; ty[0] = a.y; tz[0] = a.z;
+  tx[1] = a.w; ty[1] = b.x; tz[1] = b.y;
+  tx[2] = b.z; ty[2] = b.w; tz[2] = d.x;
+  tx[3] = d.y; ty[3] = d.z; tz[3] = d.w;
+}
 __device__ __forceinline__ void load_quad(const TermSrc &S, int64_t i0, float4 *bp, float *tx, float *ty, float *tz) {
   if (S.raw) {
 #pragma unroll
@@ -250,19 +265,7 @@
     return;
   }
   if (i0 + 3 < S.nt) {
-    if (S.pos_of) {
-      const uint4 p = *reinterpret_cast<const uint4 *>(S.pos_of + i0);
-      bp[0] = S.match[p.x]; bp[1] = S.match[p.y]; bp[2] = S.match[p.z]; bp[3] = S.match[p.w];
-    } else {
-#pragma unroll
-      for (int c = 0; c < 4; c++) bp[c] = S.match[i0 + c];
-    }
-    const float4 *x4 = reinterpret_cast<const float4 *>(S.xyz + 3 * i0);
-    const float4 a = x4[0], b = x4[1], d = x4[2];
-    tx[0] = a.x; ty[0] = a.y; tz[0] = a.z;
-    tx[1] = a.w; ty[1] = b.x; tz[1] = b.y;
-    tx[2] = b.z; ty[2] = b.w; tz[2] = d.x;
-    tx[3] = d.y; ty[3] = d.z; tz[3] = d.w;
+    load_quad_whole(S, i0, bp, tx, ty, tz);
     return;
   }
 #pragma unroll
```

After: 15350 (median of 6 runs). Within noise of the previous version (+0.8%).
